# t-taniai/LocalExpStereo

Measured on AMD Instinct MI355X. Metric: Mcost-evals/s (pixels x hypotheses / s), guided-filter cost aggregation, 1500x1000x256 vol, higher is better.
Workload: dtype i32 fixed-point box sums (exact; i64 stage-2 window sums), f32 3x3 algebra and combination

## Files before the change

localexpstereo_amd/csrc/les_hip.hip:

```cpp
#include "../../include/localexp_hip.h"
#include "les_kernels.h"
#include "les_march.h"
#include "les_propose.h"
#include "les_post.h"
#include "les_pairwise.h"
#include "les_fusion.h"
#include "les_eval.h"
#include "les_maxflow.h"
#include "les_maxflow_tiled.h"
#include "les_maxflow_cell.h"
#include "les_bilateral.h"
#include "les_vdisp.h"
#include "les_dense.h"
#include "les_costvol.h"
#include "les_crossview.h"
#include "les_wtavol.h"
#include "les_confidence.h"
#include "les_sgm.h"
#include "les_planefit.h"
#include "les_pyramid.h"
#include "les_speckle.h"
#include "les_reproject.h"

#include "../host/ResidualCut.h"

#include <algorithm>
#include <array>
#include <atomic>
#include <chrono>
#include <cmath>
#include <cstdint>
#include <mutex>
#if !defined(LES_SIM)
#include <dlfcn.h>
#endif
#include <cstdarg>
#include <cstdio>
#include <cstdlib>
#include <cstring>
#include <string>
#include <vector>

namespace {

thread_local std::string g_err;

int fail(int code, const char* fmt, ...)
{
    char buf[512];
    va_list ap;
    va_start(ap, fmt);
    vsnprintf(buf, sizeof buf, fmt, ap);
    va_end(ap);
    g_err = buf;
    return code;
}

enum FallbackReason { FB_RADIUS = 0, FB_NONFINITE, FB_RANGE, FB_THRESHOLD, FB_IMAGE_SIZE, FB_GEOMETRY, FB_PATCHES, FB_GUIDE, FB_COUNT };
void note_fallback(std::atomic<unsigned>& seen, FallbackReason r, const char* fmt, ...)
{
    if (seen.fetch_or(1u << r, std::memory_order_relaxed) & (1u << r)) return;
    static const bool quiet = [] { const char* e = getenv("LES_HIP_QUIET"); return e && atoi(e) != 0; }();
    if (quiet) return;
    char buf[512];
    va_list ap;
    va_start(ap, fmt);
    vsnprintf(buf, sizeof buf, fmt, ap);
    va_end(ap);
    fprintf(stderr, "localexp_hip: strip kernel instead of the march kernel: %s (LES_HIP_QUIET=1 silences this note)\n", buf);
}

#define HIPCHECK(expr)                                                                               \
    do {                                                                                             \
        hipError_t e_ = (expr);                                                                      \
        if (e_ != hipSuccess)                                                                        \
            return fail(LES_HIP_ERR_DEVICE, "%s failed: %s (%s:%d)", #expr, hipGetErrorString(e_), __FILE__, __LINE__); \
    } while (0)

#include "les_hip_march_tables.inc"

struct ViewData {
    float* vol = nullptr;
    bool own_vol = false;
    float4* stats = nullptr;
    uint32_t* ipk = nullptr;
    uint32_t* ipk10 = nullptr;
    float4* feat = nullptr;
    uint32_t* ipk8 = nullptr;
    float* mstats = nullptr;
    float* vol_t = nullptr;
    bool march_ok = false;
    unsigned dmax_bits = 0;
    les::MarchView mv = {};
    les::MarchView mv2 = {};
    float lo2 = 0.0f;
    bool march2_ok = false;
};

}

#include "les_hip_mem.h"

struct MtHost;
namespace { void mt_host_free(MtHost* m); }
struct WtaVol;
namespace { void wtavol_free(WtaVol* w); }
struct SgmWork;
namespace { void sgm_free(SgmWork* w); }
struct FitTables;
namespace { void fit_tables_free(FitTables* t); }

namespace {

struct VdispGroup { int c0, c1, slices; };
struct UnaryTables {
    int n = 0;
    DevBuf<char> mem;
    const les::Job* d_jobs = nullptr; int njobs = 0;
    const les::Job* d_mjobs = nullptr; int nmgroups = 0;
    const MarchEntry* mentry = nullptr;
    bool march_ok = false;
    const les::RawCall* d_rawcalls = nullptr; const long long* d_raw_off = nullptr;
    long long raw_floats = 0; int raw_chunks = 1;
    const les::WtaJob* d_targets = nullptr; const long long* d_out_off = nullptr; int out_stride = 0;
    const les::BfJob* d_bfjobs = nullptr; int nbfjobs = 0, bf_np = 1;
    std::vector<VdispGroup> vd_groups;
    const les::RawCall* d_vd_calls = nullptr;
    const float4* d_vd_stand_in = nullptr;
    int vd_max_slices = 0, vd_chunks = 1;
};

struct UnaryWorkspace {
    bool shared = false;
    struct Slot {
        DevBuf<float> raw;
        DevBuf<unsigned> flags;
        DevBuf<les::Job> rjobs;
        DevBuf<float> vol;
    } slot[2];
};

}

struct les_hip_ctx {
    les_hip_params p;
    int filter = LES_HIP_FILTER_GF;
    int R;
    DevBuf<float> d_bf_tab;
    const StripEntry* strip;
    const StripEntry* istrip[2] = {nullptr, nullptr};
    int interp = 1;
    const MarchEntry* march = nullptr;
    int ncu = 256;
    std::atomic<unsigned> fallback_seen{0};
    hipStream_t stream;
    les::Geom geom;
    ViewData v[2];
    float naive_alpha = 0;
    float naive_th_grad = 0;
    int naive = 0;
    float th_color = 0, th_grad = 0;
    float max_vdisp = 0.0f, random_vdisp = 0.0f;
    float4* d_planes = nullptr; size_t planes_cap = 0;
    DevBuf<float> d_map;
    DevBuf<les::WtaJob> d_wta;
    DevBuf<float4> d_wta_planes;
    DevBuf<float> d_pw_tab; float pw_omega = -1.f, pw_epsilon = -1.f;
    std::mutex mu;
    unsigned long long gen = 0;
    std::vector<les_hip_scratch*> idle_scratch;
    bool maxflow_lds_ready = false;
    bool maxflow_tiled_lds_ready = false;
    std::vector<les_hip_scratch*> own_scratch;
    WtaVol* wtavol = nullptr;
    SgmWork* sgm = nullptr;
    FitTables* fit_tables = nullptr;
    DevBuf<long long> mesh_ws[2];
    std::vector<MtHost*> mt_idle;
    ~les_hip_ctx()
    {
        for (ViewData& w : v) {
            if (w.own_vol && w.vol) (void)hipFree(w.vol);
            for (void* q : {(void*)w.stats, (void*)w.ipk, (void*)w.ipk10, (void*)w.feat, (void*)w.ipk8, (void*)w.mstats, (void*)w.vol_t})
                if (q) (void)hipFree(q);
        }
        if (d_planes) (void)hipFree(d_planes);
    }
};

struct les_hip_batch {
    int n = 0, R = 0;
    UnaryTables tab;
    mutable UnaryWorkspace ws;
    std::vector<les_hip_rect> targets;
    int device = 0;
    DevBuf<les::Rect4> d_units;
    DevBuf<les::WtaJob> d_targets;
    DevBuf<float> rs_disp; DevBuf<int> rs_idx, rs_noi, rs_no; DevBuf<uint64_t> rs_state; DevBuf<float> rs_refit; DevBuf<les::RansacCell> rs_cell;
    les::RansacScratch rs = {nullptr, nullptr, nullptr, nullptr, nullptr, nullptr, 0, nullptr};
    int wta_chunks = 1;
    int graph_chunks = 1;
    std::vector<long long> graph_off;
    long long graph_nodes = 0;
    DevBuf<long long> d_graph_off;
    DevBuf<double> d_flow0;
    mutable std::mutex mt_mu;
    mutable DevBuf<les::MtTile> d_mt_tiles;
    mutable DevBuf<int> d_mt_tiles_per_cell;
    mutable int mt_ntiles = -1;
    mutable std::mutex mf_mu;
    mutable DevBuf<int> d_mf_list;
    mutable int mf_list_key = -1;
    mutable int mf_count[3] = {0, 0, 0};
    mutable std::mutex re_mu;
    mutable DevBuf<double> d_region_part[2];
    mutable int region_chunks = -1;
};

struct les_hip_scratch {
    les_hip_ctx* c = nullptr;
    hipStream_t stream = nullptr;
    DevBuf<float> d_tile; PinnedBuf<float> h_tile;
    DevBuf<float4> d_plane; PinnedBuf<float4> h_plane;
    struct Entry { les_hip_rect f, t; UnaryTables tab; unsigned long long stamp; };
    std::vector<Entry> cache;
    unsigned long long clock = 0;
    UnaryWorkspace ws;
};

namespace {

std::atomic<unsigned long long> g_ctx_gen{0};
std::mutex g_live_mu;
std::vector<std::pair<unsigned long long, les_hip_ctx*>> g_live;
void release_hidden_scratch(unsigned long long gen, les_hip_scratch* s)
{
    std::lock_guard<std::mutex> lk(g_live_mu);
    for (auto& e : g_live)
        if (e.first == gen) {
            std::lock_guard<std::mutex> lk2(e.second->mu);
            e.second->idle_scratch.push_back(s);
            return;
        }
}
thread_local unsigned long long tl_stream_gen = 0;
thread_local hipStream_t tl_stream = nullptr;
inline hipStream_t cur_stream(const les_hip_ctx* c) { return (tl_stream_gen != 0 && tl_stream_gen == c->gen) ? tl_stream : c->stream; }

#include "les_hip_march.inc"

float naive_alpha(const les_hip_ctx* c) { return c->naive_alpha; }

#include "les_hip_vdisp.inc"
#include "les_hip_bilateral.inc"
#include "les_hip_unary.inc"

}

#include "les_hip_context.inc"
#include "les_hip_batch.inc"
#include "les_hip_cuts.inc"
#include "les_hip_eval.inc"
#include "les_hip_speckle.inc"
#include "les_hip_ingest_post.inc"
#include "les_hip_exchange.inc"
#include "les_hip_dense.inc"
#include "les_hip_costvol.inc"
#include "les_hip_crossview.inc"
#include "les_hip_wtavol.inc"
#include "les_hip_confidence.inc"
#include "les_hip_sgm.inc"
#include "les_hip_planefit.inc"
#include "les_hip_pyramid.inc"
#include "les_hip_reproject.inc"
```

localexpstereo_amd/csrc/les_hip_march.inc:

```
int check_rects(const les_hip_ctx* c, const les_hip_rect& f, const les_hip_rect& t)
{
    if (f.w < 0 || f.h < 0 || t.w < 0 || t.h < 0) return fail(LES_HIP_ERR_ARG, "negative rect size");
    if (f.x < 0 || f.y < 0 || f.x + f.w > c->p.W || f.y + f.h > c->p.H) return fail(LES_HIP_ERR_ARG, "filterRect outside the image");
    if (t.w > 0 && t.h > 0 && (t.x < f.x || t.y < f.y || t.x + t.w > f.x + f.w || t.y + t.h > f.y + f.h))
        return fail(LES_HIP_ERR_ARG, "targetRect not inside filterRect");
    return LES_HIP_OK;
}

int build_jobs(const les_hip_ctx* c, int n, const les_hip_rect* frs, const les_hip_rect* trs, int out_slabs,
               std::vector<les::Job>& jobs)
{
    const int TW = c->strip->TW, R = c->R;
    const long long P = (long long)c->p.H * c->p.W;
    long long strips = 0;
    for (int i = 0; i < n; i++) {
        int rc = check_rects(c, frs[i], trs[i]);
        if (rc) return rc;
        if (trs[i].w > 0 && trs[i].h > 0) strips += (trs[i].w + TW - 1) / TW;
    }
    int max_rows = 1 << 30;
    if (strips > 0 && strips < 2048) {
        long long want = (2048 + strips - 1) / strips;
        int tallest = 0;
        for (int i = 0; i < n; i++) tallest = std::max(tallest, trs[i].h);
        max_rows = std::max<long long>(std::max(8 * R, 64), (tallest + want - 1) / want);
    }
    jobs.clear();
    for (int i = 0; i < n; i++) {
        const les_hip_rect &f = frs[i], &t = trs[i];
        if (t.w <= 0 || t.h <= 0) continue;
        for (int sy = 0; sy < t.h; sy += max_rows)
            for (int sx = 0; sx < t.w; sx += TW) {
                les::Job j;
                j.tx0 = t.x + sx; j.ty0 = t.y + sy;
                j.tw = std::min(TW, t.w - sx); j.th = std::min(max_rows, t.h - sy);
                j.cx0 = f.x; j.cy0 = f.y; j.cx1 = f.x + f.w; j.cy1 = f.y + f.h;
                j.out_off = (out_slabs ? (long long)(i / out_slabs) * P : 0) + (long long)j.ty0 * c->p.W + j.tx0;
                j.out_stride = c->p.W;
                j.plane_idx = i;
                jobs.push_back(j);
            }
    }
    std::stable_sort(jobs.begin(), jobs.end(), [](const les::Job& a, const les::Job& b) {
        if (a.tx0 != b.tx0) return a.tx0 < b.tx0;
        if (a.ty0 != b.ty0) return a.ty0 < b.ty0;
        return a.plane_idx < b.plane_idx;
    });
    return LES_HIP_OK;
}

bool build_march_jobs(les_hip_ctx* c, int n, const les_hip_rect* frs, const les_hip_rect* trs, int out_slabs,
                      std::vector<les::Job>& jobs, bool& ok, const MarchEntry*& entry)
{
    jobs.clear();
    ok = false;
    entry = nullptr;
    if (!c->march) return true;
    const int R = c->R, W = c->p.W, H = c->p.H;
    const long long P = (long long)H * W;
    ok = true;
    for (int i = 0; i < n; i++) {
        const les_hip_rect &f = frs[i], &t = trs[i];
        if (t.w <= 0 || t.h <= 0) continue;
        if ((f.x > 0 && t.x - f.x < 2 * R) || (f.x + f.w < W && (f.x + f.w) - (t.x + t.w) < 2 * R) ||
            (f.y > 0 && t.y - f.y < 2 * R) || (f.y + f.h < H && (f.y + f.h) - (t.y + t.h) < 2 * R)) ok = false;
    }
    if (!ok) {
        note_fallback(c->fallback_seen, FB_GEOMETRY, "a target rectangle lies closer than 2 x radius = %d pixels to a filterRect border that is not an image border", 2 * R);
        return true;
    }
    const int ncu = c->ncu;
    const MarchEntry* cands[2] = {c->march, find_march(c->R, 0)};
    const MarchEntry* m = c->march;
    int max_rows = 1 << 30;
    {
        double best = 1e300;
        const int row_opts[] = {1 << 30, 1024, 512, 384, 256, 192, 128, 96, 64, 48, 32};
        for (int g = 0; g < 2; g++) {
            const MarchEntry* e = cands[g];
            if (!e || (g == 1 && e == cands[0])) continue;
            if (const char* w = getenv("LES_HIP_MARCH_WIDE")) if ((atoi(w) != 0) != (g == 0)) continue;
            for (int ro : row_opts) {
                long long njobs = 0;
                int rows = 0, useful = 0;
                for (int i = 0; i < n; i++) {
                    const les_hip_rect& t = trs[i];
                    if (t.w <= 0 || t.h <= 0) continue;
                    const int ns = (t.w + e->TW - 1) / e->TW;
                    const int nr = (t.h + ro - 1) / ro, sh = (t.h + nr - 1) / nr;
                    njobs += (long long)ns * nr;
                    rows = std::max(rows, sh);
                    useful = std::max(useful, (t.w + ns - 1) / ns);
                }
                if (njobs == 0) continue;
                const long long wgs = (njobs + e->NJ - 1) / e->NJ;
                const double ticks = (double)((rows + 4 * R + e->BY - 1) / e->BY + 3);
                const double cost = (double)((wgs + ncu - 1) / ncu) * ticks * (1.0 + 1e-3 * (double)wgs / ncu) + (ro == (1 << 30) ? 0.0 : 1e-6);
                if (cost < best) { best = cost; m = e; max_rows = ro; }
            }
        }
    }
    if (const char* e = getenv("LES_HIP_MARCH_ROWS")) max_rows = std::max(1, atoi(e));
    entry = m;
    const int TW = m->TW, NJ = m->NJ;
    for (int i = 0; i < n; i++) {
        const les_hip_rect &f = frs[i], &t = trs[i];
        if (t.w <= 0 || t.h <= 0) continue;
        const int ns = (t.w + TW - 1) / TW, sw = (t.w + ns - 1) / ns;
        const int nr = (t.h + max_rows - 1) / max_rows, sh = (t.h + nr - 1) / nr;
        for (int sy = 0; sy < t.h; sy += sh)
            for (int sx = 0; sx < t.w; sx += sw) {
                les::Job j;
                j.tx0 = t.x + sx; j.ty0 = t.y + sy;
                j.tw = std::min(sw, t.w - sx); j.th = std::min(sh, t.h - sy);
                j.cx0 = f.x; j.cy0 = f.y; j.cx1 = f.x + f.w; j.cy1 = f.y + f.h;
                j.out_off = (out_slabs ? (long long)(i / out_slabs) * P : 0) + (long long)j.ty0 * W + j.tx0;
                j.out_stride = W;
                j.plane_idx = i;
                jobs.push_back(j);
            }
    }
    std::stable_sort(jobs.begin(), jobs.end(), [](const les::Job& a, const les::Job& b) {
        if (a.tx0 != b.tx0) return a.tx0 < b.tx0;
        if (a.ty0 != b.ty0) return a.ty0 < b.ty0;
        return a.plane_idx < b.plane_idx;
    });
    while (!jobs.empty() && jobs.size() % NJ) {
        les::Job pad = jobs.back();
        pad.tw = 0; pad.th = 0;
        jobs.push_back(pad);
    }
    return true;
}

int ensure_planes(les_hip_ctx* c, size_t n)
{
    if (n <= c->planes_cap) return LES_HIP_OK;
    if (c->d_planes) HIPCHECK(hipFree(c->d_planes));
    c->d_planes = nullptr; c->planes_cap = 0;
    size_t cap = std::max<size_t>(n, 1024);
    HIPCHECK(hipMalloc((void**)&c->d_planes, cap * sizeof(float4)));
    c->planes_cap = cap;
    return LES_HIP_OK;
}

struct RawPatches { const les::RawCall* calls; const long long* off; float* raw; int n, chunks; };

les::View strip_view(const les_hip_ctx* c, int mode)
{
    les::View view{c->v[mode].vol, c->v[mode].stats, c->v[mode].ipk, c->v[mode].ipk10, nullptr, nullptr, mode ? -1.0f : 1.0f, c->th_color, c->th_grad};
    if (c->naive) { view.feat_self = c->v[mode].feat; view.feat_other = c->v[1 - mode].feat; }
    return view;
}

int launch_march(les_hip_ctx* c, const MarchEntry* m, int mode, const les::Job* d_mjobs, int ngroups, const float4* d_planes, float* d_out, int check,
                 hipStream_t stream, const RawPatches* rp = nullptr)
{
    if (ngroups <= 0) return LES_HIP_OK;
    les::MarchView mv = c->v[mode].mv;
    if (c->naive) {
        if (!rp || !rp->raw || !c->v[1 - mode].feat) return fail(LES_HIP_ERR_ARG, "view %d was not supplied at creation", mode);
        hipLaunchKernelGGL(les::les_naive_raw_kernel, dim3(rp->n, rp->chunks), dim3(256), 0, stream, c->geom, strip_view(c, mode), rp->calls, d_planes, rp->raw);
        mv.vol = rp->raw; mv.raw_off = rp->off;
    }
    hipLaunchKernelGGL(m->fn, dim3(ngroups), dim3(m->NT), 0, stream, c->geom, mv, d_mjobs, d_planes, d_out, ngroups, check);
    HIPCHECK(hipGetLastError());
    return LES_HIP_OK;
}

const StripEntry* strip_for(const les_hip_ctx* c) { return (c->naive || c->interp == 1) ? c->strip : c->istrip[c->interp == 0 ? 0 : 1]; }

int launch_strips(les_hip_ctx* c, int mode, const les::Job* d_jobs, int njobs, const float4* d_planes, float* d_out, int check, hipStream_t stream)
{
    if (njobs <= 0) return LES_HIP_OK;
    if (mode < 0 || mode > 1 || !c->v[mode].stats || (c->naive ? !c->v[1 - mode].feat : !c->v[mode].vol))
        return fail(LES_HIP_ERR_ARG, "view %d was not supplied at creation", mode);
    const StripEntry* se = strip_for(c);
    if (!se) return fail(LES_HIP_ERR_UNSUPPORTED, "no strip kernel for interpolation %d at guided-filter radius %d", c->interp, c->R);
    const les::View view = strip_view(c, mode);
    hipLaunchKernelGGL(se->fn, dim3(njobs), dim3(se->NT), 0, stream, c->geom, view, d_jobs, d_planes, d_out, njobs, check);
    HIPCHECK(hipGetLastError());
    return LES_HIP_OK;
}

bool interp_march_ok(const les_hip_ctx* c, int mode)
{
    return !c->naive && c->interp != 1 && c->march && c->v[mode].march_ok && (c->interp == 0 || c->v[mode].march2_ok);
}

int launch_nan_spread(les_hip_ctx* c, int mode, int n, const les::RawCall* calls, const les::WtaJob* targets, const long long* out_off, int stride,
                      const float4* d_planes, const unsigned* flags, float* d_out, int check, hipStream_t stream)
{
    if (n <= 0) return LES_HIP_OK;
    if (c->interp == 2)
        hipLaunchKernelGGL(les::les_nan_spread_kernel<2>, dim3(n), dim3(256), 0, stream, c->geom, (const float*)c->v[mode].vol, calls, targets, out_off, stride,
                           d_planes, flags, d_out, 2 * c->R, check);
    else
        hipLaunchKernelGGL(les::les_nan_spread_kernel<0>, dim3(n), dim3(256), 0, stream, c->geom, (const float*)c->v[mode].vol, calls, targets, out_off, stride,
                           d_planes, flags, d_out, 2 * c->R, check);
    HIPCHECK(hipGetLastError());
    return LES_HIP_OK;
}

int launch_interp_march(les_hip_ctx* c, const MarchEntry* m, int mode, const les::Job* d_mjobs, int ngroups, const RawPatches& rp,
                        unsigned* d_flags, const les::Job* d_sjobs, les::Job* d_rjobs, int nsjobs, const les::WtaJob* targets, const long long* out_off,
                        int stride, const float4* d_planes, float* d_out, int check, hipStream_t stream)
{
    const ViewData& v = c->v[mode];
    const bool quad = c->interp == 2;
    les::MarchView mv = quad ? v.mv2 : v.mv;
    mv.vol = rp.raw; mv.raw_off = rp.off; mv.vol_t = nullptr;
    if (quad) {
        if (!c->istrip[1]) return fail(LES_HIP_ERR_UNSUPPORTED, "no strip kernel for interpolation 2 at guided-filter radius %d", c->R);
        HIPCHECK(hipMemsetAsync(d_flags, 0, (size_t)rp.n * sizeof(unsigned), stream));
        hipLaunchKernelGGL(les::les_interp_raw_kernel<2>, dim3(rp.n, rp.chunks), dim3(256), 0, stream, c->geom, (const float*)v.vol, rp.calls, d_planes,
                           rp.raw, d_flags, v.lo2);
    } else {
        hipLaunchKernelGGL(les::les_interp_raw_kernel<0>, dim3(rp.n, rp.chunks), dim3(256), 0, stream, c->geom, (const float*)v.vol, rp.calls, d_planes,
                           rp.raw, (unsigned*)nullptr, -INFINITY);
    }
    HIPCHECK(hipGetLastError());
    if (ngroups > 0) hipLaunchKernelGGL(m->fn, dim3(ngroups), dim3(m->NT), 0, stream, c->geom, mv, d_mjobs, d_planes, d_out, ngroups, check);
    HIPCHECK(hipGetLastError());
    if (quad && nsjobs > 0) {
        hipLaunchKernelGGL(les::les_mask_jobs_kernel, dim3((nsjobs + 255) / 256), dim3(256), 0, stream, d_sjobs, d_rjobs, (const unsigned*)d_flags, nsjobs);
        HIPCHECK(hipGetLastError());
        const StripEntry* se = c->istrip[1];
        hipLaunchKernelGGL(se->fn, dim3(nsjobs), dim3(se->NT), 0, stream, c->geom, strip_view(c, mode), (const les::Job*)d_rjobs, d_planes, d_out, nsjobs, check);
        HIPCHECK(hipGetLastError());
        return launch_nan_spread(c, mode, rp.n, rp.calls, targets, out_off, stride, d_planes, d_flags, d_out, check, stream);
    }
    return LES_HIP_OK;
}

float naive_alpha(const les_hip_ctx* c);

int build_march_view(les_hip_ctx* c, int m, const double* d_hs)
{
    ViewData& v = c->v[m];
    const size_t P = (size_t)c->p.H * c->p.W;
    const int W = c->p.W, H = c->p.H;
    v.march_ok = false;
    v.march2_ok = false;
    if ((unsigned long long)P * (4ull * les::kMarchStatWords) >= (1ull << 31)) {
        note_fallback(c->fallback_seen, FB_IMAGE_SIZE, "image of %d x %d pixels (32-bit row offsets reach 2^26 pixels)", W, H);
        return LES_HIP_OK;
    }
    const float th = c->naive ? c->th_color + c->th_grad : c->p.th_col;
    if (!(th > 0.0f) || !(th < INFINITY)) { note_fallback(c->fallback_seen, FB_THRESHOLD, "truncation threshold %g is not positive and finite", (double)th); return LES_HIP_OK; }
    if (d_hs) {
        unsigned dbits = 0;
        struct DevBuf { void* p = nullptr; ~DevBuf() { if (p) (void)hipFree(p); } } dm;
        HIPCHECK(hipMalloc(&dm.p, sizeof(unsigned)));
        unsigned* d_dmax = static_cast<unsigned*>(dm.p);
        HIPCHECK(hipMemsetAsync(d_dmax, 0, sizeof(unsigned), cur_stream(c)));
        HIPCHECK(hipMalloc((void**)&v.ipk8, P * sizeof(uint32_t)));
        HIPCHECK(hipMalloc((void**)&v.mstats, P * les::kMarchStatWords * sizeof(float)));
        hipLaunchKernelGGL(les::les_march_stats_kernel, dim3((W + 255) / 256, H), dim3(256), 0, cur_stream(c), d_hs, v.ipk, v.ipk8, v.mstats, d_dmax, H, W, c->R, c->p.eps);
        HIPCHECK(hipGetLastError());
        HIPCHECK(hipMemcpyAsync(&dbits, d_dmax, sizeof(unsigned), hipMemcpyDeviceToHost, cur_stream(c)));
        HIPCHECK(hipStreamSynchronize(cur_stream(c)));
        v.dmax_bits = dbits;
    }
    auto drop_tiled = [&]() { if (v.vol_t) { (void)hipFree(v.vol_t); v.vol_t = nullptr; } };
    const int nb = 2048;
    std::vector<float> hmin(nb, 0.0f); std::vector<int> hbad(nb, 0);
    if (!c->naive) {
        struct DevBuf { void* p = nullptr; ~DevBuf() { if (p) (void)hipFree(p); } } part;
        HIPCHECK(hipMalloc(&part.p, nb * (sizeof(float) + sizeof(int))));
        float* d_min = static_cast<float*>(part.p);
        int* d_bad = reinterpret_cast<int*>(d_min + nb);
        hipLaunchKernelGGL(les::les_range_kernel, dim3(nb), dim3(256), 0, cur_stream(c), v.vol, P * (size_t)c->p.D, d_min, d_bad);
        HIPCHECK(hipGetLastError());
        HIPCHECK(hipMemcpyAsync(hmin.data(), d_min, nb * sizeof(float), hipMemcpyDeviceToHost, cur_stream(c)));
        HIPCHECK(hipMemcpyAsync(hbad.data(), d_bad, nb * sizeof(int), hipMemcpyDeviceToHost, cur_stream(c)));
        HIPCHECK(hipStreamSynchronize(cur_stream(c)));
    }
    float vmin = INFINITY; int bad = 0;
    for (int i = 0; i < nb; i++) { vmin = std::min(vmin, hmin[i]); bad |= hbad[i]; }
    if (bad || !(vmin < INFINITY)) {
        note_fallback(c->fallback_seen, FB_NONFINITE, "the cost volume of view %d holds NaN or infinite entries", m);
        drop_tiled();
        return LES_HIP_OK;
    }
    vmin = std::min(vmin, 0.5f * th);
    const double range = (double)th - (double)vmin;
    if (!(range <= 8.0 * (double)th)) {
        note_fallback(c->fallback_seen, FB_RANGE, "view %d: costs reach %g below the truncation threshold %g (more than 8 x the threshold)", m, range, (double)th);
        drop_tiled();
        return LES_HIP_OK;
    }
    const unsigned dbits = v.dmax_bits;
    float dmax;
    memcpy(&dmax, &dbits, sizeof dmax);
    if (!(dmax > 0.0f) || !(dmax < INFINITY)) { note_fallback(c->fallback_seen, FB_GUIDE, "view %d: the inverse covariance of the guide is not positive and finite (largest diagonal entry %g)", m, (double)dmax); return LES_HIP_OK; }
    const int K = 2 * c->R + 1;
    auto scaled_view = [&](float lo) {
        const double range = (double)th - (double)lo;
        const double Ba = 0.5 * range * std::sqrt((double)dmax), Bb = range + 1.5 * Ba;
        const double scale = 1073741824.0 / ((double)K * Bb * 1.25);
        const int PB = les::march_pb(c->R);
        const float spf = (float)((double)((1 << PB) - 1) / range);
        const double c0 = std::rint(-(double)lo * (double)spf) - (double)(1 << (PB - 1));
        const double up = 1.0 / (double)spf;
        les::MarchView mv;
        mv.vol = v.vol; mv.ipk8 = v.ipk8; mv.mstats = v.mstats;
        mv.sp = spf;
        mv.pmagic = (float)(12582912.0 + c0);
        mv.poff = (float)(-c0 * up);
        mv.kapS = (float)((double)(1 << les::kMarchSH) * up / 255.0 * scale);
        mv.upS = (float)(up * scale);
        mv.qscale = (float)((double)(1 << les::kMarchS2) / (255.0 * scale));
        mv.kmu = (float)(1.0 / ((double)(1ll << les::kMarchMB) * 255.0));
        mv.raw_off = nullptr;
        mv.vol_t = nullptr;
        return mv;
    };
    les::MarchView mv = scaled_view(vmin);
    if (!c->naive) {
        const float lo2 = (float)((double)vmin - 0.5 * range);
        if ((double)th - (double)lo2 <= 8.0 * (double)th) {
            v.mv2 = scaled_view(lo2);
            v.lo2 = lo2;
            v.march2_ok = true;
        }
    }
    if (!c->naive && v.vol) {
        const char* e = getenv("LES_HIP_TILED");
        const unsigned long long nt = (unsigned long long)H * (unsigned long long)((W + 7) / 8) * 8ull * (unsigned long long)c->p.D;
        if (!(e && atoi(e) == 0) && (unsigned long long)((W + 7) / 8) * (unsigned long long)c->p.D * 32ull < (1ull << 31)) {
            if (v.vol_t) { (void)hipFree(v.vol_t); v.vol_t = nullptr; }
            size_t mem_free = 0, mem_total = 0;
            const bool room = hipMemGetInfo(&mem_free, &mem_total) == hipSuccess && mem_free >= 2 * nt * sizeof(float) + (4ull << 30);
            if (room && hipMalloc((void**)&v.vol_t, nt * sizeof(float)) == hipSuccess) {
                hipLaunchKernelGGL(les::les_tile_volume_kernel, dim3((unsigned)(((W + 7) / 8 * 8 + 63) / 64), (unsigned)H), dim3(256), 0, cur_stream(c), v.vol, v.vol_t, c->p.D, H, W);
                HIPCHECK(hipGetLastError());
                mv.vol_t = v.vol_t;
            } else {
                (void)hipGetLastError();
                v.vol_t = nullptr;
            }
        }
    }
    v.mv = mv;
    v.march_ok = true;
    return LES_HIP_OK;
}

int build_view(les_hip_ctx* c, int m, const uint8_t* im, const float* vol)
{
    const size_t P = (size_t)c->p.H * c->p.W;
    ViewData& v = c->v[m];
    if (vol) {
        if (c->p.volumes_on_device) { v.vol = const_cast<float*>(vol); v.own_vol = false; }
        else {
            HIPCHECK(hipMalloc((void**)&v.vol, P * c->p.D * sizeof(float)));
            v.own_vol = true;
            HIPCHECK(hipMemcpy(v.vol, vol, P * c->p.D * sizeof(float), hipMemcpyHostToDevice));
        }
    }
    if (!im) return LES_HIP_OK;
    uint8_t* d_img = nullptr;
    double* d_hs = nullptr;
    HIPCHECK(hipMalloc((void**)&d_img, P * 3));
    HIPCHECK(hipMemcpy(d_img, im, P * 3, hipMemcpyHostToDevice));
    HIPCHECK(hipMalloc((void**)&v.ipk, P * sizeof(uint32_t)));
    HIPCHECK(hipMalloc((void**)&v.ipk10, P * sizeof(uint32_t)));
    HIPCHECK(hipMalloc((void**)&v.stats, (P * 3 + 1) * sizeof(float4)));
    HIPCHECK(hipMemsetAsync(v.stats + P * 3, 0, sizeof(float4), cur_stream(c)));
    HIPCHECK(hipMalloc((void**)&d_hs, P * 9 * sizeof(double)));
    const int W = c->p.W, H = c->p.H;
    if (c->naive) {
        HIPCHECK(hipMalloc((void**)&v.feat, P * sizeof(float4)));
        hipLaunchKernelGGL(les::les_naive_features_kernel, dim3((c->p.W + 255) / 256, c->p.H), dim3(256), 0, cur_stream(c), d_img, v.feat, c->p.H, c->p.W, naive_alpha(c));
    }
    hipLaunchKernelGGL(les::les_pack_guide_kernel, dim3((unsigned)((P + 255) / 256)), dim3(256), 0, cur_stream(c), d_img, v.ipk, v.ipk10, (int)P);
    hipLaunchKernelGGL(les::les_stats_hsum_kernel, dim3((W + 255) / 256, H), dim3(256), 0, cur_stream(c), v.ipk, d_hs, H, W, c->R);
    hipLaunchKernelGGL(les::les_stats_finish_kernel, dim3((W + 255) / 256, H), dim3(256), 0, cur_stream(c), d_hs, v.stats, H, W, c->R, c->p.eps);
    HIPCHECK(hipGetLastError());
    if (c->march && (v.vol || c->naive)) {
        int rc = build_march_view(c, m, d_hs);
        if (rc) { (void)hipFree(d_img); (void)hipFree(d_hs); return rc; }
    }
    HIPCHECK(hipStreamSynchronize(cur_stream(c)));
    HIPCHECK(hipFree(d_img));
    HIPCHECK(hipFree(d_hs));
    return LES_HIP_OK;
}
```

localexpstereo_amd/csrc/les_hip_march_tables.inc:

```
typedef void (*StripKernel)(les::Geom, les::View, const les::Job*, const float4*, float*, int, int);
struct StripEntry { int R; int variant; int TW; int NT; StripKernel fn; };

#define LES_STRIP_ENTRY(R_, V_, WA_, BY_, SEG_, MW_) \
    { R_, V_, les::StripCfg<R_, WA_, BY_, SEG_>::TW, les::StripCfg<R_, WA_, BY_, SEG_>::NT, les::les_strip_kernel<R_, WA_, BY_, SEG_, MW_> }
const StripEntry kStrips[] = {
    LES_STRIP_ENTRY(1, 0, 64, 16, 4, 2), LES_STRIP_ENTRY(2, 0, 64, 16, 4, 2), LES_STRIP_ENTRY(3, 0, 64, 16, 4, 2),
    LES_STRIP_ENTRY(4, 0, 64, 16, 4, 2), LES_STRIP_ENTRY(5, 0, 64, 16, 4, 2), LES_STRIP_ENTRY(6, 0, 64, 16, 4, 2),
    LES_STRIP_ENTRY(7, 0, 64, 16, 4, 2), LES_STRIP_ENTRY(8, 0, 64, 16, 4, 2), LES_STRIP_ENTRY(9, 0, 64, 16, 4, 2),
    LES_STRIP_ENTRY(10, 0, 64, 21, 3, 3), LES_STRIP_ENTRY(12, 0, 64, 16, 4, 2), LES_STRIP_ENTRY(15, 0, 96, 16, 6, 2),
    LES_STRIP_ENTRY(10, 8, 128, 21, 6, 2), LES_STRIP_ENTRY(10, 11, 64, 21, 3, 2),
};
#define LES_NAIVE_ENTRY(R_, WA_, BY_, SEG_, MW_) \
    { R_, 0, les::StripCfg<R_, WA_, BY_, SEG_>::TW, les::StripCfg<R_, WA_, BY_, SEG_>::NT, les::les_strip_kernel<R_, WA_, BY_, SEG_, MW_, 1> }
const StripEntry kNaiveStrips[] = {
    LES_NAIVE_ENTRY(1, 64, 16, 4, 2), LES_NAIVE_ENTRY(2, 64, 16, 4, 2), LES_NAIVE_ENTRY(3, 64, 16, 4, 2), LES_NAIVE_ENTRY(4, 64, 16, 4, 2),
    LES_NAIVE_ENTRY(5, 64, 16, 4, 2), LES_NAIVE_ENTRY(6, 64, 16, 4, 2), LES_NAIVE_ENTRY(7, 64, 16, 4, 2), LES_NAIVE_ENTRY(8, 64, 16, 4, 2),
    LES_NAIVE_ENTRY(9, 64, 16, 4, 2), LES_NAIVE_ENTRY(10, 64, 16, 4, 2), LES_NAIVE_ENTRY(12, 64, 16, 4, 2), LES_NAIVE_ENTRY(15, 96, 16, 6, 2),
};
#define LES_INTERP_ENTRY(R_, WA_, BY_, SEG_, MW_, SRC_) \
    { R_, 0, les::StripCfg<R_, WA_, BY_, SEG_>::TW, les::StripCfg<R_, WA_, BY_, SEG_>::NT, les::les_strip_kernel<R_, WA_, BY_, SEG_, MW_, SRC_> }
#define LES_INTERP_ENTRIES(SRC_) \
    LES_INTERP_ENTRY(1, 64, 16, 4, 2, SRC_), LES_INTERP_ENTRY(2, 64, 16, 4, 2, SRC_), LES_INTERP_ENTRY(3, 64, 16, 4, 2, SRC_), \
    LES_INTERP_ENTRY(4, 64, 16, 4, 2, SRC_), LES_INTERP_ENTRY(5, 64, 16, 4, 2, SRC_), LES_INTERP_ENTRY(6, 64, 16, 4, 2, SRC_), \
    LES_INTERP_ENTRY(7, 64, 16, 4, 2, SRC_), LES_INTERP_ENTRY(8, 64, 16, 4, 2, SRC_), LES_INTERP_ENTRY(9, 64, 16, 4, 2, SRC_), \
    LES_INTERP_ENTRY(10, 64, 16, 4, 2, SRC_), LES_INTERP_ENTRY(12, 64, 16, 4, 2, SRC_), LES_INTERP_ENTRY(15, 96, 16, 6, 2, SRC_)
const StripEntry kNearestStrips[] = { LES_INTERP_ENTRIES(2) };
const StripEntry kQuadraticStrips[] = { LES_INTERP_ENTRIES(3) };
const StripEntry* find_interp_strip(int R, int interp)
{
    for (const auto& e : (interp == 0 ? kNearestStrips : kQuadraticStrips))
        if (e.R == R) return &e;
    return nullptr;
}
const StripEntry* find_naive_strip(int R)
{
    for (const auto& e : kNaiveStrips)
        if (e.R == R) return &e;
    return nullptr;
}
const StripEntry* find_strip(int R)
{
    int variant = 0;
    if (const char* v = getenv("LES_HIP_VARIANT")) variant = atoi(v);
    const StripEntry* def = nullptr;
    for (const auto& e : kStrips) {
        if (e.R != R) continue;
        if (e.variant == variant) return &e;
        if (e.variant == 0) def = &e;
    }
    return def;
}

typedef void (*MarchKernel)(les::Geom, les::MarchView, const les::Job*, const float4*, float*, int, int);
struct MarchEntry { int R; int TW; int NJ; int NT; int BY; MarchKernel fn; };
#define LES_MARCH_ENTRY(R_, WGC_, NJ_, BY_) \
    { R_, les::MarchCfg<R_, WGC_, NJ_, BY_>::TW, NJ_, les::MarchCfg<R_, WGC_, NJ_, BY_>::NT, BY_, les::les_march_kernel<R_, WGC_, NJ_, BY_> }
const MarchEntry kMarch[] = {
    LES_MARCH_ENTRY(10, 256, 1, 7),
#if defined(LES_MARCH_LAB) && defined(LES_MARCH_NARROW_NJ1)
    LES_MARCH_ENTRY(10, 128, 1, 7),
#else
    LES_MARCH_ENTRY(10, 128, 2, 7),
#endif
    LES_MARCH_ENTRY(7, 256, 1, 5),
    LES_MARCH_ENTRY(7, 128, 2, 5),
#if !defined(LES_MARCH_FEW_RADII)
    LES_MARCH_ENTRY(2, 256, 1, 2),  LES_MARCH_ENTRY(2, 128, 2, 2),
    LES_MARCH_ENTRY(3, 256, 1, 3),  LES_MARCH_ENTRY(3, 128, 2, 3),
    LES_MARCH_ENTRY(4, 256, 1, 3),  LES_MARCH_ENTRY(4, 128, 2, 3),
    LES_MARCH_ENTRY(5, 256, 1, 4),  LES_MARCH_ENTRY(5, 128, 2, 4),
    LES_MARCH_ENTRY(6, 256, 1, 5),  LES_MARCH_ENTRY(6, 128, 2, 5),
    LES_MARCH_ENTRY(8, 256, 1, 6),  LES_MARCH_ENTRY(8, 128, 2, 6),
    LES_MARCH_ENTRY(9, 256, 1, 7),  LES_MARCH_ENTRY(9, 128, 2, 7),
#endif
};
const MarchEntry* find_march(int R, int wide = 1)
{
    if (const char* k = getenv("LES_HIP_KERNEL")) if (!strcmp(k, "strip")) return nullptr;
    const MarchEntry* best = nullptr;
    for (const auto& e : kMarch)
        if (e.R == R && (!best || (wide ? e.TW > best->TW : e.TW < best->TW))) best = &e;
    return best;
}

constexpr long long kRawPatchCapFloats = 1ll << 30;
constexpr int kRansacMaxSam = 500;
constexpr int kRansacChunks = 5;
constexpr int kRansacChunkEnds[kRansacChunks] = {16, 64, 128, 256, kRansacMaxSam};
```

localexpstereo_amd/csrc/les_hip_unary.inc:

```

int build_unary_tables(les_hip_ctx* c, int n, const les_hip_rect* frs, const les_hip_rect* trs, int out_slabs, bool compact, UnaryTables& t)
{
    for (int i = 0; i < n; i++) {
        int rc = check_rects(c, frs[i], trs[i]);
        if (rc) return rc;
    }
    t.n = n;
    const long long P = (long long)c->p.H * c->p.W;
    std::vector<les::RawCall> calls((size_t)n);
    std::vector<long long> raw_off((size_t)n), out_off((size_t)n);
    long long amax = 1;
    for (int i = 0; i < n; i++) {
        const les_hip_rect &f = frs[i], &r = trs[i];
        const bool live = r.w > 0 && r.h > 0;
        const long long a = live ? (long long)f.w * f.h : 0;
        calls[i] = les::RawCall{f.x, f.y, live ? f.w : 0, live ? f.h : 0, t.raw_floats};
        raw_off[i] = t.raw_floats;
        out_off[i] = compact ? 0 : (out_slabs ? (long long)(i / out_slabs) * P : 0) + (long long)r.y * c->p.W + r.x;
        t.raw_floats += a; amax = std::max(amax, a);
    }
    t.raw_chunks = (int)std::min<long long>(1024, std::max<long long>(1, (amax + 4095) / 4096));
    t.out_stride = compact ? trs[0].w : c->p.W;
    std::vector<les::Job> jobs, mjobs;
    std::vector<les::BfJob> bfjobs;
    std::vector<les::RawCall> vd_calls;
    std::vector<float4> vd_stand;
    if (c->filter == LES_HIP_FILTER_GF) {
        int rc = build_jobs(c, n, frs, trs, out_slabs, jobs);
        if (rc) return rc;
        bool mok = false;
        build_march_jobs(c, n, frs, trs, out_slabs, mjobs, mok, t.mentry);
        t.march_ok = mok && !mjobs.empty();
        if (t.march_ok && c->naive && t.raw_floats > kRawPatchCapFloats) {
            t.march_ok = false;
            note_fallback(c->fallback_seen, FB_PATCHES, "the raw-cost patches of one batch of the image-based energy exceed 4 GB");
        }
        if (!t.march_ok) mjobs.clear();
        if (compact)
            for (auto* v : {&jobs, &mjobs})
                for (les::Job& j : *v) { j.out_off = (long long)(j.ty0 - trs[0].y) * trs[0].w + (j.tx0 - trs[0].x); j.out_stride = trs[0].w; }
        if (c->naive) vdisp_layout(c, n, frs, trs, t, vd_calls, vd_stand);
    } else {
        if (t.raw_floats > kRawPatchCapFloats)
            return fail(LES_HIP_ERR_UNSUPPORTED, "the raw-cost patches of one batch exceed 4 GB (%lld floats): split the batch", t.raw_floats);
        int rc = build_bf_jobs(c, n, frs, trs, out_slabs, compact, bfjobs, t.bf_np);
        if (rc) return rc;
    }
    t.njobs = (int)jobs.size();
    t.nmgroups = t.march_ok ? (int)(mjobs.size() / t.mentry->NJ) : 0;
    t.nbfjobs = (int)bfjobs.size();
    std::vector<char> blob;
    auto put = [&](const auto& v) -> size_t {
        if (v.empty()) return SIZE_MAX;
        const size_t off = (blob.size() + 255) & ~(size_t)255, bytes = v.size() * sizeof(v[0]);
        blob.resize(off + bytes);
        memcpy(blob.data() + off, v.data(), bytes);
        return off;
    };
    static_assert(sizeof(les::WtaJob) == sizeof(les_hip_rect), "rect layout");
    const std::vector<les_hip_rect> targets(trs, trs + n);
    const size_t o_jobs = put(jobs), o_mjobs = put(mjobs), o_calls = put(calls), o_raw_off = put(raw_off), o_targets = put(targets),
                 o_out_off = put(out_off), o_bfjobs = put(bfjobs), o_vd_calls = put(vd_calls), o_vd_stand = put(vd_stand);
    if (blob.empty()) return LES_HIP_OK;
    int rc = t.mem.alloc(blob.size());
    if (rc) return rc;
    HIPCHECK(hipMemcpy(t.mem.p, blob.data(), blob.size(), hipMemcpyHostToDevice));
    auto at = [&](size_t off) -> const void* { return off == SIZE_MAX ? nullptr : t.mem.p + off; };
    t.d_jobs = static_cast<const les::Job*>(at(o_jobs));
    t.d_mjobs = static_cast<const les::Job*>(at(o_mjobs));
    t.d_rawcalls = static_cast<const les::RawCall*>(at(o_calls));
    t.d_raw_off = static_cast<const long long*>(at(o_raw_off));
    t.d_targets = static_cast<const les::WtaJob*>(at(o_targets));
    t.d_out_off = static_cast<const long long*>(at(o_out_off));
    t.d_bfjobs = static_cast<const les::BfJob*>(at(o_bfjobs));
    t.d_vd_calls = static_cast<const les::RawCall*>(at(o_vd_calls));
    t.d_vd_stand_in = static_cast<const float4*>(at(o_vd_stand));
    return LES_HIP_OK;
}

int unary_kind(const les_hip_ctx* c, const UnaryTables& t, int mode)
{
    if (c->filter != LES_HIP_FILTER_GF) return 2;
    if (!t.march_ok) return 0;
    if (c->naive || c->interp == 1) return c->march && c->v[mode].march_ok ? 1 : 0;
    return interp_march_ok(c, mode) && t.raw_floats <= kRawPatchCapFloats ? 1 : 0;
}

int run_unary(les_hip_ctx* c, const UnaryTables& t, UnaryWorkspace& w, int mode, const float4* d_planes, float* d_out, int check, hipStream_t stream)
{
    int rc = view_ok(c, mode);
    if (rc) return rc;
    const int kind = unary_kind(c, t, mode);
    const bool patches = kind == 2 || (kind == 1 && (c->naive || c->interp != 1));
    const bool vdisp = kind == 0 && c->naive;
    const bool masked = vdisp || (kind == 1 && !c->naive && c->interp == 2);
    UnaryWorkspace::Slot& s = w.slot[w.shared ? mode : 0];
    if (patches || masked) {
        std::unique_lock<std::mutex> lk(c->mu, std::defer_lock);
        if (w.shared) lk.lock();
        const size_t min_raw = w.shared ? 1 : 256 * 256, min_jobs = w.shared ? 1 : 64;
        if (patches) rc = s.raw.grow((size_t)std::max<long long>(t.raw_floats, 1), min_raw, stream);
        if (!rc && masked) rc = s.flags.grow((size_t)std::max(t.n, 1), 1, stream);
        if (!rc && masked) rc = s.rjobs.grow((size_t)std::max(t.njobs, 1), min_jobs, stream);
        if (!rc && vdisp) rc = s.vol.grow(std::max<size_t>((size_t)t.vd_max_slices * c->p.H * c->p.W, 1), 1, stream);
        if (rc) return rc;
    }
    const RawPatches rp{t.d_rawcalls, t.d_raw_off, s.raw.p, t.n, t.raw_chunks};
    if (kind == 2) return launch_bf(c, mode, t.d_bfjobs, t.nbfjobs, t.bf_np, t.d_rawcalls, t.n, t.raw_chunks, s.raw.p, d_planes, d_out, check, stream);
    if (kind == 1) {
        if (c->naive) return launch_naive_march(c, t.mentry, mode, t.d_mjobs, t.nmgroups, d_planes, d_out, check, stream, rp);
        if (c->interp == 1) return launch_march(c, t.mentry, mode, t.d_mjobs, t.nmgroups, d_planes, d_out, check, stream);
        return launch_interp_march(c, t.mentry, mode, t.d_mjobs, t.nmgroups, rp, s.flags.p, t.d_jobs, s.rjobs.p, t.njobs, t.d_targets, t.d_out_off,
                                   t.out_stride, d_planes, d_out, check, stream);
    }
    if (!c->naive && c->interp != 1 && t.march_ok && interp_march_ok(c, mode))
        note_fallback(c->fallback_seen, FB_PATCHES, "the raw-cost patches of one batch at interpolation %d exceed 4 GB", c->interp);
    rc = launch_strips(c, mode, t.d_jobs, t.njobs, d_planes, d_out, check, stream);
    if (rc) return rc;
    if (vdisp) return launch_vdisp_strips(c, t, s.vol.p, s.flags.p, s.rjobs.p, mode, d_planes, d_out, check, stream);
    if (!c->naive && c->interp != 1)
        return launch_nan_spread(c, mode, t.n, t.d_rawcalls, t.d_targets, t.d_out_off, t.out_stride, d_planes, nullptr, d_out, check, stream);
    return LES_HIP_OK;
}
```

localexpstereo_amd/csrc/les_hip_vdisp.inc:

```

void launch_naive_raw(les_hip_ctx* c, int mode, const les::RawCall* calls, int n, int chunks, const float4* d_planes, float* raw, hipStream_t stream)
{
    hipLaunchKernelGGL(les::les_naive_raw_v_kernel, dim3(n, chunks), dim3(256), 0, stream, c->geom, strip_view(c, mode), calls, d_planes, raw, 0, 0,
                       (unsigned*)nullptr);
}

int launch_naive_march(les_hip_ctx* c, const MarchEntry* m, int mode, const les::Job* d_mjobs, int ngroups, const float4* d_planes, float* d_out, int check,
                       hipStream_t stream, const RawPatches& rp)
{
    if (ngroups <= 0) return LES_HIP_OK;
    if (!rp.raw || !c->v[1 - mode].feat) return fail(LES_HIP_ERR_ARG, "view %d was not supplied at creation", mode);
    launch_naive_raw(c, mode, rp.calls, rp.n, rp.chunks, d_planes, rp.raw, stream);
    les::MarchView mv = c->v[mode].mv;
    mv.vol = rp.raw; mv.raw_off = rp.off;
    hipLaunchKernelGGL(m->fn, dim3(ngroups), dim3(m->NT), 0, stream, c->geom, mv, d_mjobs, d_planes, d_out, ngroups, check);
    HIPCHECK(hipGetLastError());
    return LES_HIP_OK;
}

constexpr long long kVdispVolCapFloats = 1ll << 28;

void vdisp_layout(const les_hip_ctx* c, int n, const les_hip_rect* frs, const les_hip_rect* trs, UnaryTables& t, std::vector<les::RawCall>& calls,
                  std::vector<float4>& stand)
{
    const long long HW = (long long)c->p.H * c->p.W;
    const int cap = (int)std::max<long long>(1, kVdispVolCapFloats / std::max<long long>(HW, 1));
    calls.resize((size_t)n);
    stand.resize((size_t)n);
    std::vector<std::vector<les_hip_rect>> used;
    VdispGroup g{0, 0, 0};
    long long amax = 1;
    for (int i = 0; i < n; i++) {
        const les_hip_rect f = frs[i];
        const bool live = trs[i].w > 0 && trs[i].h > 0 && f.w > 0 && f.h > 0;
        int s = 0;
        if (live) {
            auto overlaps = [&](const les_hip_rect& r) { return f.x < r.x + r.w && r.x < f.x + f.w && f.y < r.y + r.h && r.y < f.y + f.h; };
            for (s = 0; s < (int)used.size(); s++) {
                bool free_ = true;
                for (const auto& r : used[s]) if (overlaps(r)) { free_ = false; break; }
                if (free_) break;
            }
            if (s == (int)used.size()) {
                if (s == cap) {
                    g.c1 = i; g.slices = s; t.vd_groups.push_back(g);
                    g = VdispGroup{i, i, 0};
                    used.clear(); s = 0;
                }
                used.emplace_back();
            }
            used[s].push_back(f);
            amax = std::max(amax, (long long)f.w * f.h);
        }
        calls[i] = les::RawCall{f.x, f.y, live ? f.w : 0, live ? f.h : 0, (long long)s * HW + (long long)f.y * c->p.W + f.x};
        stand[i] = make_float4(0.0f, 0.0f, (float)s, 0.0f);
    }
    g.c1 = n; g.slices = (int)used.size(); t.vd_groups.push_back(g);
    for (const auto& gg : t.vd_groups) t.vd_max_slices = std::max(t.vd_max_slices, gg.slices);
    t.vd_chunks = (int)std::min<long long>(1024, std::max<long long>(1, (amax + 4095) / 4096));
}

int launch_vdisp_strips(les_hip_ctx* c, const UnaryTables& t, float* vol, unsigned* flags, les::Job* rjobs, int mode, const float4* d_planes,
                        float* d_out, int check, hipStream_t stream)
{
    const int njobs = t.njobs;
    if (njobs <= 0 || t.n <= 0 || t.vd_max_slices <= 0) return LES_HIP_OK;
    const StripEntry* se = find_interp_strip(c->R, 0);
    if (!se || se->TW < c->strip->TW)
        return fail(LES_HIP_ERR_UNSUPPORTED, "no nearest-slice strip kernel for guided-filter radius %d (vertical disparity on the strip path)", c->R);
    les::Geom g = c->geom;
    g.D0 = 0; g.th_col = INFINITY;
    les::View view = strip_view(c, mode);
    view.vol = vol;
    const les::RawCall* vd_calls = t.d_vd_calls;
    const les::Job* jobs = t.d_jobs;
    const float4* stand_in = t.d_vd_stand_in;
    for (const auto& gr : t.vd_groups) {
        if (gr.c1 <= gr.c0 || gr.slices <= 0) continue;
        g.D = gr.slices;
        if (t.vd_groups.size() > 1) HIPCHECK(hipMemsetAsync(flags, 0, (size_t)t.n * sizeof(unsigned), stream));
        hipLaunchKernelGGL(les::les_naive_raw_v_kernel, dim3(gr.c1 - gr.c0, t.vd_chunks), dim3(256), 0, stream, c->geom, strip_view(c, mode),
                           vd_calls + gr.c0, d_planes + gr.c0, vol, c->p.W, 1, flags + gr.c0);
        hipLaunchKernelGGL(les::les_mask_jobs_kernel, dim3((njobs + 255) / 256), dim3(256), 0, stream, jobs, rjobs, (const unsigned*)flags, njobs);
        hipLaunchKernelGGL(se->fn, dim3(njobs), dim3(se->NT), 0, stream, g, view, (const les::Job*)rjobs, stand_in, d_out, njobs, 0);
        if (check)
            hipLaunchKernelGGL(les::les_vdisp_check_kernel, dim3(njobs), dim3(256), 0, stream, c->geom, (const les::Job*)rjobs, d_planes, d_out, njobs);
        HIPCHECK(hipGetLastError());
    }
    return LES_HIP_OK;
}
```

localexpstereo_amd/csrc/les_march.h:

```cpp
#pragma once

#include "les_kernels.h"

#if defined(LES_MARCH_LAB)
#include "les_march_lab.h"
#else
#define LES_MARCH_ROLE_ORDER 5
#define LES_STATS_POLICY ""
#define LES_LAB_ROLE_ON(bit) true
#define LES_LAB_ABLATE(bit) false
#endif
#ifndef LES_TICK_BEGIN
#define LES_TICK_BEGIN() ((void)0)
#define LES_TICK_MARK() ((void)0)
#define LES_TICK_BARRIER() __syncthreads()
#define LES_TICK_END(role_) ((void)0)
#endif

namespace les {

constexpr int kMarchSH = 5;
constexpr int kMarchMB = 24;
constexpr int kMarchSL = 3;
constexpr int kMarchS2 = 4;
constexpr int kMarchMagicBits = 0x4B400000;
static_assert(kMarchSH + kMarchMB + kMarchSL == 32, "N cov = t - hi32(M * (s << SL)) needs the scales to meet at 2^32");
__host__ __device__ constexpr int march_pb(int R) { return (2 * R + 1) * (2 * R + 1) < 512 ? 20 : 19; }
#ifndef LES_MARCH_STAT_WORDS
#define LES_MARCH_STAT_WORDS 9
#endif
constexpr int kMarchStatWords = LES_MARCH_STAT_WORDS;
static_assert(kMarchStatWords == 9 || kMarchStatWords == 12, "statistics record of 36 or 48 bytes");

struct MarchView {
    const float* vol;
    const uint32_t* ipk8;
    const float* mstats;
    float sp;
    float pmagic;
    float poff;
    float kapS;
    float upS;
    float qscale;
    float kmu;
    const long long* raw_off;
    const float* vol_t;
};
#ifndef LES_TILED_MIN_SLOPE_WIDE
#define LES_TILED_MIN_SLOPE_WIDE 0.05f
#endif
#ifndef LES_TILED_MIN_SLOPE
#define LES_TILED_MIN_SLOPE 0.125f
#endif

template <int R, int WGC, int NJ, int BY>
struct MarchCfg {
    static constexpr int KS = 2 * R + 1;
    static constexpr int RS = 3 * BY;
    static constexpr int TW = WGC - 4 * R;
    static constexpr int HWV = WGC / 64;
    static constexpr int NW = 3 * HWV * NJ;
    static constexpr int NT = 64 * NW;
    static constexpr int SEGL = 8;
    static constexpr int PADW = 16;
    static constexpr int PCOLS0 = 1 + WGC + WGC / PADW;
    static constexpr int PCOLS = PCOLS0 + ((4 - PCOLS0 % 8) + 8) % 8;
    static_assert(RS >= KS, "the ring must hold a whole window (the row that leaves it is the one written KS rows ago)");
    static_assert(RS - KS < BY, "a ring longer than the window by a block or more wastes registers: pick the smallest block height");
    static_assert(WGC % 64 == 0, "a job slot is a whole number of waves");
    static_assert(BY * (64 / SEGL) <= 64, "one wave prefixes its own tile");
    static_assert(TW > 0, "job too narrow for this radius");
    static_assert(2 * R + 1 < 64, "a window crosses at most one wave boundary");
    static_assert((long long)KS * KS * (1ll << (march_pb(R) - 1 + kMarchSL)) < (1ll << 31), "stage-1 window sums (shifted for the product with M) must fit int32");
    static_assert((long long)KS * 128 * (1ll << (march_pb(R) - 1)) < (1ll << 31), "vertical sums of Iq * pi must fit int32");
    static_assert((long long)KS * (1ll << (30 - kMarchS2)) < (1ll << 31), "the stage-2 window sums, rounded to 2^S2, must fit int32");
    __host__ __device__ static constexpr int pcol(int ci) { return 1 + ci + ci / PADW; }
};

__device__ __forceinline__ void march_prefix_scan8(int4 (&v)[8])
{
#pragma unroll
    for (int j = 1; j < 8; j++) { v[j].x += v[j - 1].x; v[j].y += v[j - 1].y; v[j].z += v[j - 1].z; v[j].w += v[j - 1].w; }
    int4 inc = v[7];
#if defined(LES_SIM) || defined(LES_MARCH_SCAN_PLAIN)
#define LES_SCAN_STEP(N) { inc.x += dpp_row_shr<N>(inc.x); inc.y += dpp_row_shr<N>(inc.y); inc.z += dpp_row_shr<N>(inc.z); inc.w += dpp_row_shr<N>(inc.w); }
    LES_SCAN_STEP(2) LES_SCAN_STEP(4) LES_SCAN_STEP(8)
#undef LES_SCAN_STEP
#else
#define LES_SCAN_ROW(N) "v_add_u32_dpp %0, %0, %0 row_shr:" #N " row_mask:0xf bank_mask:0xf bound_ctrl:1\n" \
                        "v_add_u32_dpp %1, %1, %1 row_shr:" #N " row_mask:0xf bank_mask:0xf bound_ctrl:1\n" \
                        "v_add_u32_dpp %2, %2, %2 row_shr:" #N " row_mask:0xf bank_mask:0xf bound_ctrl:1\n" \
                        "v_add_u32_dpp %3, %3, %3 row_shr:" #N " row_mask:0xf bank_mask:0xf bound_ctrl:1\n"
    asm("s_nop 1\n" LES_SCAN_ROW(2) LES_SCAN_ROW(4) LES_SCAN_ROW(8) : "+v"(inc.x), "+v"(inc.y), "+v"(inc.z), "+v"(inc.w));
#undef LES_SCAN_ROW
#endif
    const int4 off = int4{inc.x - v[7].x, inc.y - v[7].y, inc.z - v[7].z, inc.w - v[7].w};
#pragma unroll
    for (int j = 0; j < 8; j++) { v[j].x += off.x; v[j].y += off.y; v[j].z += off.z; v[j].w += off.w; }
}

template <int BY, int PCOLS>
__device__ __forceinline__ void march_prefix_tile(int4 (*T)[PCOLS], int ci0, int lane)
{
    constexpr int SEGL = 8;
    const int row = 2 * (lane >> 4) + (lane & 1), seg = (lane & 15) >> 1;
    const bool act = row < BY;
    const int c0 = ci0 + seg * SEGL;
    int4* p = &T[act ? row : 0][1 + c0 + c0 / 16];
    int4 v[SEGL];
#pragma unroll
    for (int j = 0; j < SEGL; j++) v[j] = p[j];
    march_prefix_scan8(v);
    if (act) {
#pragma unroll
        for (int j = 0; j < SEGL; j++) lds_store4(&p[j], v[j].x, v[j].y, v[j].z, v[j].w);
    }
}

template <int BY, int PCOLS>
__device__ __forceinline__ void march_prefix_pair(int4 (*TA)[PCOLS], int4 (*TB)[PCOLS], int ci0, int lane)
{
    constexpr int SEGL = 8;
    const int row = 2 * (lane >> 4) + (lane & 1), seg = (lane & 15) >> 1;
    const bool act = row < BY;
    const int c0 = ci0 + seg * SEGL;
    const int pc = 1 + c0 + c0 / 16;
    int4* pa = &TA[act ? row : 0][pc];
    int4* pb = &TB[act ? row : 0][pc];
    int4 va[SEGL], vb[SEGL];
#pragma unroll
    for (int j = 0; j < SEGL; j++) vb[j] = pb[j];
    wave_sync();
#pragma unroll
    for (int j = 0; j < SEGL; j++) va[j] = pa[j];
    LES_MARCH_SCHED_FENCE();
    march_prefix_scan8(vb);
    if (act) {
#pragma unroll
        for (int j = 0; j < SEGL; j++) lds_store4(&pb[j], vb[j].x, vb[j].y, vb[j].z, vb[j].w);
    }
    LES_MARCH_SCHED_FENCE();
    march_prefix_scan8(va);
    if (act) {
#pragma unroll
        for (int j = 0; j < SEGL; j++) lds_store4(&pa[j], va[j].x, va[j].y, va[j].z, va[j].w);
    }
}

#if defined(LES_SIM)
typedef float4 mstat4;
#else
typedef float mstat4 __attribute__((ext_vector_type(4)));
#endif
#if LES_MARCH_STAT_WORDS == 9
typedef float mstat_tail;
#else
typedef mstat4 mstat_tail;
#endif
struct MarchStatRow { mstat4 a, b; mstat_tail c; };
#if defined(LES_SIM) || defined(LES_MARCH_STATS_PLAIN)
struct MarchStatDesc { const char* base; uint32_t bytes; };
__device__ inline MarchStatDesc march_stats_desc(const float* base, uint32_t bytes) { return MarchStatDesc{(const char*)base, bytes}; }
__device__ inline void march_stats_load(MarchStatRow& r, const MarchStatDesc& d, uint32_t voff, uint32_t soff)
{
    const unsigned long long o = (unsigned long long)voff + (unsigned long long)soff;
    float w[8 + sizeof(mstat_tail) / 4];
    for (unsigned i = 0; i < sizeof w / 4; i++) w[i] = (o + 4ull * i + 4 <= d.bytes) ? *reinterpret_cast<const float*>(d.base + o + 4ull * i) : 0.0f;
    memcpy(&r.a, w, 16); memcpy(&r.b, w + 4, 16); memcpy(&r.c, w + 8, sizeof r.c);
}
template <int N>
__device__ inline void march_stats_wait(MarchStatRow& r) { (void)r; }
template <int N>
__device__ inline void march_stats_wait(MarchStatRow& r, MarchStatRow& q) { (void)r; (void)q; }
#else
typedef int MarchStatDesc __attribute__((ext_vector_type(4)));
__device__ __forceinline__ MarchStatDesc march_stats_desc(const float* base, uint32_t bytes)
{
    const unsigned long long a = (unsigned long long)base;
    MarchStatDesc d;
    d.x = __builtin_amdgcn_readfirstlane((int)(uint32_t)a);
    d.y = __builtin_amdgcn_readfirstlane((int)((uint32_t)(a >> 32) & 0xffffu));
    d.z = __builtin_amdgcn_readfirstlane((int)bytes);
    d.w = 0x00027000;
    return d;
}
__device__ __forceinline__ void march_stats_load(MarchStatRow& r, const MarchStatDesc& d, uint32_t voff, uint32_t soff)
{
    asm volatile("buffer_load_dwordx4 %0, %1, %2, %3 offen" LES_STATS_POLICY : "+v"(r.a) : "v"(voff), "s"(d), "s"(soff));
    asm volatile("buffer_load_dwordx4 %0, %1, %2, %3 offen offset:16" LES_STATS_POLICY : "+v"(r.b) : "v"(voff), "s"(d), "s"(soff));
#if LES_MARCH_STAT_WORDS == 9
    asm volatile("buffer_load_dword %0, %1, %2, %3 offen offset:32" LES_STATS_POLICY : "+v"(r.c) : "v"(voff), "s"(d), "s"(soff));
#else
    asm volatile("buffer_load_dwordx4 %0, %1, %2, %3 offen offset:32" LES_STATS_POLICY : "+v"(r.c) : "v"(voff), "s"(d), "s"(soff));
#endif
}
template <int N>
__device__ __forceinline__ void march_stats_wait(MarchStatRow& r) { asm volatile("s_waitcnt vmcnt(%3)" : "+v"(r.a), "+v"(r.b), "+v"(r.c) : "n"(N)); }
template <int N>
__device__ __forceinline__ void march_stats_wait(MarchStatRow& r, MarchStatRow& q)
{
    asm volatile("s_waitcnt vmcnt(%6)" : "+v"(r.a), "+v"(r.b), "+v"(r.c), "+v"(q.a), "+v"(q.b), "+v"(q.c) : "n"(N));
}
#endif
__device__ __forceinline__ int march_stat_m2(const MarchStatRow& r)
{
#if LES_MARCH_STAT_WORDS == 9
    return __float_as_int(r.c);
#else
    return __float_as_int(r.c.x);
#endif
}

__device__ __forceinline__ bool march_label_surely_valid(const Geom& g, float4 pl, int x0, int x1, int y0, int y1)
{
    const float ax0 = pl.x * (float)x0, ax1 = pl.x * (float)x1, by0 = pl.y * (float)y0, by1 = pl.y * (float)y1;
    const float spread = 5.0f * (fabsf(pl.x) + fabsf(pl.y));
    const float lo = (fminf(ax0, ax1) + fminf(by0, by1)) + pl.z - spread;
    const float hi = (fmaxf(ax0, ax1) + fmaxf(by0, by1)) + pl.z + spread;
    const float mag = fmaxf(fabsf(ax0), fabsf(ax1)) + fmaxf(fabsf(by0), fabsf(by1)) + fabsf(pl.z) + spread;
    const float margin = 1e-5f * mag + 1e-30f;
    return (0.0f * pl.w == 0.0f) && mag < 1e30f && (lo - margin >= g.mind) && (hi + margin <= g.maxd);
}

__device__ __forceinline__ bool march_plane_short_gather(const Geom& g, float4 pl, const Job& job, int R, int* slice_lo)
{
    *slice_lo = 0;
    const unsigned long long HW = (unsigned long long)g.H * (unsigned long long)g.W;
    const bool moderate = fabsf(pl.x) < 1e30f && fabsf(pl.y) < 1e30f && fabsf(pl.z) < 1e30f;
    if (!(moderate && g.mind == 0.0f && g.D0 == 0 && g.maxd == (float)(g.D - 1) && g.D >= 2 && HW < (1ull << 24))) return false;
    if ((unsigned long long)g.D * HW < (1ull << 30)) return true;
    const int x0 = max(job.tx0 - 2 * R, job.cx0), x1 = min(job.tx0 + job.tw + 2 * R, job.cx1) - 1;
    const int y0 = max(job.ty0 - 2 * R, job.cy0), y1 = min(job.ty0 + job.th + 2 * R, job.cy1) - 1;
    if (x1 < x0 || y1 < y0) return false;
    const float ax0 = pl.x * (float)x0, ax1 = pl.x * (float)x1, by0 = pl.y * (float)y0, by1 = pl.y * (float)y1;
    const float lo = (fminf(ax0, ax1) + fminf(by0, by1)) + pl.z, hi = (fmaxf(ax0, ax1) + fmaxf(by0, by1)) + pl.z;
    const float mag = fmaxf(fabsf(ax0), fabsf(ax1)) + fmaxf(fabsf(by0), fabsf(by1)) + fabsf(pl.z);
    const float margin = 1e-5f * mag + 1e-30f;
    if (!((lo - margin >= 0.0f) && (hi + margin < g.maxd))) return false;
    const int s0 = (int)floorf(lo - margin), s1 = (int)floorf(hi + margin) + 1;
    *slice_lo = s0;
    return s0 >= 0 && s1 < g.D && (unsigned long long)(s1 - s0 + 1) * HW < (1ull << 28);
}

template <int R, int WGC, int NJ, int BY>
__global__ void __launch_bounds__(3 * WGC * NJ)
les_march_kernel(Geom g, MarchView view, const Job* __restrict__ jobs, const float4* __restrict__ planes,
                 float* __restrict__ out, int ngroups, int check)
{
    using Cfg = MarchCfg<R, WGC, NJ, BY>;
    constexpr int KS = Cfg::KS, RS = Cfg::RS, NT = Cfg::NT, HWV = Cfg::HWV, PCOLS = Cfg::PCOLS;
    constexpr int UN = 3;

    __shared__ int4 s_T1[2][NJ][BY][PCOLS];
    __shared__ int4 s_T2[3][NJ][BY][PCOLS];
    __shared__ float s_rtab[KS + 1];

    int grp;
    {
        const int nwg = (int)gridDim.x, orig = (int)blockIdx.x;
        const int q = nwg / 8, r = nwg % 8, xcd = orig % 8;
        grp = (xcd < r ? xcd * (q + 1) : r * (q + 1) + (xcd - r) * q) + orig / 8;
    }
    if (grp >= ngroups) return;
    const int tid = (int)threadIdx.x;
    const int lane = tid & 63;
    const int wave = readfirstlane_i32(tid >> 6);
    constexpr int kRoleOf[6][3] = {{0, 1, 2}, {2, 1, 0}, {1, 2, 0}, {2, 0, 1}, {1, 0, 2}, {0, 2, 1}};
    const int slot = wave / (3 * HWV), role = kRoleOf[LES_MARCH_ROLE_ORDER][(wave % (3 * HWV)) / HWV], half = wave % HWV;
    const int ci0 = half * 64, ci = ci0 + lane;
    const Job job = jobs[grp * NJ + slot];
    int th_max = 0;
#pragma unroll
    for (int s = 0; s < NJ; s++) th_max = max(th_max, jobs[grp * NJ + s].th);
    const int nblk = (th_max + 4 * R + BY - 1) / BY;
    const int nticks = nblk + 3;
    const int Ttot = job.th > 0 ? job.th + 4 * R : 0;
    const float4 plane = planes[job.plane_idx];
    const int cy1m = max(job.cy1 - 1, job.cy0);

    if (tid <= KS) s_rtab[tid] = tid > 0 ? (float)(1.0 / (double)tid) : 0.0f;
    for (int k = tid; k < 3 * NJ * BY; k += NT) {
        if (k < 2 * NJ * BY) (&s_T1[0][0][0][0])[k * PCOLS] = int4{0, 0, 0, 0};
        (&s_T2[0][0][0][0])[k * PCOLS] = int4{0, 0, 0, 0};
    }
    __syncthreads();

    const int gx = job.tx0 - 2 * R + ci;
    const bool col_in = gx >= job.cx0 && gx < job.cx1 && job.th > 0;
    const int sx = min(max(gx, job.cx0), max(job.cx1 - 1, job.cx0));
    const uint32_t sx4 = (uint32_t)sx * 4u;
    const uint32_t rowB = (uint32_t)g.W * 4u;
    const uint32_t imgB = (uint32_t)g.H * rowB;
    const BufRsrc rs_guide = make_buf(view.ipk8, imgB);
    const int nx = window_count(gx, R, job.cx0, job.cx1);
    const int cP = min(ci + R, WGC - 1), cM = ci - R - 1;
    const int pcP = Cfg::pcol(cP);
    const int pcM = cM >= 0 ? Cfg::pcol(cM) : 0;
    const bool cross = cM >= 0 && (cP >> 6) != (cM >> 6);
    const int pcX = cross ? Cfg::pcol((cP >> 6) * 64 - 1) : 0;
    const int pcS = Cfg::pcol(ci);

    if (role == 0 && LES_LAB_ROLE_ON(1)) {
        const uint32_t HWu = (uint32_t)g.H * (uint32_t)g.W;
        const float g_ax = plane.x * (float)sx;
        const bool fronto = plane.x == 0.0f && plane.y == 0.0f;
        GatherPrep gpc = gather_prepare(g, 0.0f, plane.z, 0u, HWu, true);
        if (gpc.f1 == 0.0f) gpc.i1 = gpc.i0;
        int ringN[RS];
        uint32_t ringG[RS];
#pragma unroll
        for (int k = 0; k < RS; k++) { ringN[k] = 0; ringG[k] = 0u; }
        int Sp = 0;
        int Sc[3] = {1 << (kMarchSH - 1), 1 << (kMarchSH - 1), 1 << (kMarchSH - 1)};
        const uint32_t i0s = (uint32_t)readfirstlane_i32((int)gpc.i0), i1s = (uint32_t)readfirstlane_i32((int)gpc.i1);
        const float f1s = __int_as_float(readfirstlane_i32(__float_as_int(gpc.f1)));
        const int modes = readfirstlane_i32(gpc.mode);
        const float f0s = 1.0f - f1s;
        const bool inv_job = fronto && modes == 2 && !view.raw_off;
        int slice_lo = 0;
        const bool tame = !fronto && !view.raw_off && march_plane_short_gather(g, plane, job, R, &slice_lo);
        const uint32_t W8 = ((uint32_t)g.W + 7u) >> 3;
        const uint32_t trowB = W8 * (uint32_t)g.D * 32u;
        const int trow_lo = max(job.ty0 - 2 * R, job.cy0);
        const int trow_hi = min(job.ty0 - 2 * R + (nblk + 2) * BY, job.cy1);
        const unsigned long long tspanB = (unsigned long long)max(trow_hi - trow_lo, 1) * (unsigned long long)trowB;
        const bool tiled = tame && view.vol_t && fabsf(plane.x) >= (NJ == 1 ? LES_TILED_MIN_SLOPE_WIDE : LES_TILED_MIN_SLOPE) && tspanB < 0xfffffff0ull &&
                           (unsigned long long)W8 * (unsigned long long)g.D * 32ull < (1ull << 31);
        const float spj = !col_in ? 0.0f : (inv_job ? 0.0f : view.sp);
        const float pmj = !col_in ? __int_as_float(kMarchMagicBits) : (inv_job ? fmaf(g.th_col, view.sp, view.pmagic) : view.pmagic);
        auto march_a = [&](auto kind_tag) __attribute__((always_inline)) {
        constexpr int KIND = decltype(kind_tag)::value;
        GatherPrep gp[BY];
        float v0[BY], v1[BY];
        float f1r[BY];
        uint32_t gw[BY];
        uint32_t rowbits = 0, rowbits_nx = 0;
        int nx_rowB = 0;
        float nx_dbase = 0.0f;
        int nx_rowraw = 0;
        int nx_rowT = 0;
        const int fw = job.cx1 - job.cx0;
        const float* v0base = view.vol + (size_t)i0s;
        if constexpr (KIND == 3) v0base = view.vol + view.raw_off[job.plane_idx] - job.cx0;
        if constexpr (KIND == 4) v0base = view.vol + (size_t)slice_lo * (size_t)HWu;
        if constexpr (KIND == 5) v0base = view.vol_t + (size_t)trow_lo * (size_t)(trowB >> 2);
        const unsigned long long rest4 = (unsigned long long)(g.D - slice_lo) * (unsigned long long)imgB;
        const unsigned long long trestB = (unsigned long long)(g.H - trow_lo) * (unsigned long long)trowB;
        const uint32_t tiledB = (uint32_t)(trestB < 0xfffffffcull ? trestB : 0xfffffffcull);
        const BufRsrc rs_v0 = make_buf(v0base, KIND == 3 ? 0xfffffffcu : (KIND == 4 ? (uint32_t)(rest4 < 0xfffffffcull ? rest4 : 0xfffffffcull) : (KIND == 5 ? tiledB : imgB)));
        const uint32_t tcol = (((uint32_t)sx >> 3) * (uint32_t)g.D * 8u + ((uint32_t)sx & 7u)) * 4u;
        const int dsub = g.D0 - slice_lo;
        const BufRsrc rs_v1 = make_buf(view.vol + (size_t)i1s, imgB);
        auto prep = [&](int b) __attribute__((always_inline)) {
            const int t = b * BY + lane;
            const int gy = job.ty0 - 2 * R + t;
            const int sy = min(max(gy, job.cy0), cy1m);
            nx_rowB = (int)((uint32_t)sy * rowB);
            rowbits_nx = ballot_low(t < Ttot && gy >= job.cy0 && gy < job.cy1, BY);
            if constexpr (KIND == 3) nx_rowraw = (sy - job.cy0) * fw * 4;
            else nx_dbase = plane.y * (float)sy + plane.z;
            if constexpr (KIND == 5) nx_rowT = (int)((uint32_t)(sy - trow_lo) * trowB);
        };
        auto issue_row = [&](auto itag) __attribute__((always_inline)) {
            constexpr int i = decltype(itag)::value;
            const uint32_t ro = (uint32_t)readlane_i32(nx_rowB, i);
            if (LES_LAB_ABLATE(64)) { v0[i] = (float)lane; v1[i] = 0.0f; gw[i] = (uint32_t)lane; return; }
            if constexpr (KIND == 3) {
                v0[i] = buf_load<float>(rs_v0, sx4, (uint32_t)readlane_i32(nx_rowraw, i));
            } else if constexpr (KIND < 2) {
                v0[i] = buf_load<float>(rs_v0, sx4, ro);
                if constexpr (KIND == 1) v1[i] = buf_load<float>(rs_v1, sx4, ro);
            } else if constexpr (KIND == 4) {
                const float d = g_ax + readlane_f32(nx_dbase, i);
                const float dc = med3_f32(d, 0.0f, g.maxd);
                const float df = floorf(dc);
                f1r[i] = dc - df;
                const uint32_t e = mad_u24((int)df + dsub, (int)HWu, sx);
                v0[i] = buf_load<float>(rs_v0, e << 2, ro);
                v1[i] = buf_load<float>(rs_v0, (e << 2) + (f1r[i] > 0.0f ? imgB : 0u), ro);
            } else if constexpr (KIND == 5) {
                const float d = g_ax + readlane_f32(nx_dbase, i);
                const float dc = med3_f32(d, 0.0f, g.maxd);
                const float df = floorf(dc);
                f1r[i] = dc - df;
                const uint32_t e = (((uint32_t)(int)df + (uint32_t)g.D0) << 5) + tcol;
                const uint32_t rt = (uint32_t)readlane_i32(nx_rowT, i);
                v0[i] = buf_load<float>(rs_v0, e, rt);
                v1[i] = buf_load<float>(rs_v0, e + (f1r[i] > 0.0f ? 32u : 0u), rt);
            } else {
                const float d_base = readlane_f32(nx_dbase, i);
                const bool inside = col_in && ((rowbits_nx >> i) & 1u);
                gp[i] = gather_prepare(g, g_ax, d_base, (ro >> 2) + (uint32_t)sx, HWu, inside);
                if (gp[i].f1 == 0.0f) gp[i].i1 = gp[i].i0;
                v0[i] = view.vol[gp[i].i0];
                v1[i] = view.vol[gp[i].i1];
            }
            gw[i] = buf_load<uint32_t>(rs_guide, sx4, ro);
        };
        prep(0);
        rowbits = rowbits_nx;
        prep(0);
        static_for<BY>([&](auto itag) { issue_row(itag); });
        LES_TICK_BEGIN();
        for (int k0 = 0; k0 < nticks; k0 += UN) {
            static_for<UN>([&](auto utag) {
                constexpr int BASE = decltype(utag)::value * BY;
                const int k = k0 + decltype(utag)::value;
                if (k < nticks) {
                    if (k < nblk) {
                        int4 (*T)[PCOLS] = s_T1[k & 1][slot];
                        prep(k + 1);
                        static_for<BY>([&](auto itag) {
                            constexpr int i = decltype(itag)::value;
                            constexpr int SLOT = BASE + i;
                            constexpr int OLD = (SLOT + RS - KS) % RS;
                            int pi;
                            if constexpr (KIND == 3) {
                                pi = (__float_as_int(fmaf(v0[i], spj, pmj)) - kMarchMagicBits) & sbfe1(rowbits, i);
                            } else if constexpr (KIND < 2) {
                                float C = v0[i];
                                if constexpr (KIND == 1) C = f0s * v0[i] + f1s * v1[i];
                                const float p = min_f32_finite(C, g.th_col);
                                pi = (__float_as_int(fmaf(p, spj, pmj)) - kMarchMagicBits) & sbfe1(rowbits, i);
                            } else if constexpr (KIND == 4 || KIND == 5) {
                                const float f0 = 1.0f - f1r[i];
                                const float C = f0 * v0[i] + f1r[i] * v1[i];
                                const float p = min_f32_finite(C, g.th_col);
                                pi = (__float_as_int(fmaf(p, spj, pmj)) - kMarchMagicBits) & sbfe1(rowbits, i);
                            } else {
                                const float p = gather_finish(g, gp[i], v0[i], v1[i]);
                                pi = __float_as_int(fmaf(p, view.sp, view.pmagic)) - kMarchMagicBits;
                                pi = gp[i].mode == 3 ? 0 : pi;
                            }
                            const uint32_t gi = gw[i];
                            const int no = ringN[OLD];
                            const uint32_t go = ringG[OLD];
                            ringN[SLOT] = -pi;
                            ringG[SLOT] = gi;
                            Sp = Sp + pi + no;
                            Sc[0] = Sc[0] + mul24_sbyte<0>(gi, pi) + mul24_sbyte<0>(go, no);
                            Sc[1] = Sc[1] + mul24_sbyte<1>(gi, pi) + mul24_sbyte<1>(go, no);
                            Sc[2] = Sc[2] + mul24_sbyte<2>(gi, pi) + mul24_sbyte<2>(go, no);
                            lds_store4(&T[i][pcS], Sp, Sc[0] >> kMarchSH, Sc[1] >> kMarchSH, Sc[2] >> kMarchSH);
                            issue_row(itag);
                        });
                        rowbits = rowbits_nx;
                        LES_TICK_MARK();
                    }
                    {
                        int4 (*TB)[PCOLS] = s_T2[(decltype(utag)::value + UN - 2 % UN) % UN][slot];
                        const bool da = k < nblk, db = !(NJ > 1 && KIND == 2) && k >= 2 && k < nblk + 2;
                        constexpr bool kPair = KIND != 2 && KIND != 4 && KIND != 5;
                        if (kPair && da && db) march_prefix_pair<BY, PCOLS>(s_T1[k & 1][slot], TB, ci0, lane);
                        else {
                            if (da) { wave_sync(); march_prefix_tile<BY, PCOLS>(s_T1[k & 1][slot], ci0, lane); }
                            if (db) march_prefix_tile<BY, PCOLS>(TB, ci0, lane);
                        }
                    }
                    LES_TICK_BARRIER();
                }
            });
        }
        LES_TICK_END(0);
        };
        if (view.raw_off) march_a(std::integral_constant<int, 3>{});
        else if (fronto && f1s == 0.0f) march_a(std::integral_constant<int, 0>{});
        else if (fronto) march_a(std::integral_constant<int, 1>{});
        else if (tiled) march_a(std::integral_constant<int, 5>{});
        else if (tame) march_a(std::integral_constant<int, 4>{});
        else march_a(std::integral_constant<int, 2>{});
    } else if (role == 1 && LES_LAB_ROLE_ON(2)) {
        const bool s1_col = col_in && ci >= R && ci < WGC - R;
        int slice_lo_unused = 0;
        const bool general_plane = !view.raw_off && !(plane.x == 0.0f && plane.y == 0.0f) && !march_plane_short_gather(g, plane, job, R, &slice_lo_unused);
        const float kap_x = s1_col ? view.kapS * s_rtab[nx] : 0.0f;
        const float up_x = s1_col ? view.upS * s_rtab[nx] : 0.0f;
        const uint32_t sxS = (uint32_t)sx * (uint32_t)(4 * kMarchStatWords);
        const uint32_t rowS = (uint32_t)g.W * (uint32_t)(4 * kMarchStatWords);
        const MarchStatDesc ds_stats = march_stats_desc(view.mstats, (uint32_t)g.H * rowS);
        MarchStatRow st[BY];
#pragma unroll
        for (int i = 0; i < BY; i++) {
            st[i].a = st[i].b = mstat4{0.0f, 0.0f, 0.0f, 0.0f};
#if LES_MARCH_STAT_WORDS == 9
            st[i].c = 0.0f;
#else
            st[i].c = mstat4{0.0f, 0.0f, 0.0f, 0.0f};
#endif
        }
        float rny[BY];
        int nx_srow = 0;
        float nx_rny = 0.0f;
        auto prep = [&](int b) __attribute__((always_inline)) {
            const int t = b * BY + lane;
            const int gy1 = job.ty0 - 3 * R + t;
            const bool on = gy1 >= job.cy0 && gy1 < job.cy1 && t >= 2 * R && t < Ttot;
            nx_rny = on ? s_rtab[window_count(gy1, R, job.cy0, job.cy1)] : 0.0f;
            nx_srow = (int)((uint32_t)min(max(gy1, job.cy0), cy1m) * rowS);
        };
        auto issue_row = [&](auto itag) __attribute__((always_inline)) {
            constexpr int i = decltype(itag)::value;
            rny[i] = readlane_f32(nx_rny, i);
            uint32_t soff = (uint32_t)readlane_i32(nx_srow, i) & 0xfffffffcu;
            if (LES_LAB_ABLATE(4)) soff &= 0x3u;
            if (LES_LAB_ABLATE(1)) return;
            march_stats_load(st[i], ds_stats, sxS, soff);
        };
        prep(0);
        static_for<BY>([&](auto itag) { issue_row(itag); });
        LES_TICK_BEGIN();
        for (int k = 0; k < nticks; k++) {
            if (k >= 1 && k <= nblk) {
                const int b = k - 1;
                const int4 (*T1)[PCOLS] = s_T1[b & 1][slot];
                int4 (*T2)[PCOLS] = s_T2[b % 3][slot];
                constexpr int GC = 2, NS = (BY + GC - 1) / GC;
                prep(k);
                int4 pp[2][GC], pm[2][GC], px[2][GC];
                auto lds_stage = [&](auto stag) __attribute__((always_inline)) {
                    constexpr int S = decltype(stag)::value;
#pragma unroll
                    for (int j = 0; j < GC; j++)
                        if (S * GC + j < BY) {
                            if (LES_LAB_ABLATE(2)) { pp[S & 1][j] = int4{lane, k, 2, 3}; pm[S & 1][j] = int4{3, 2, k, lane}; px[S & 1][j] = int4{0, 0, 0, 0}; }
                            else { pp[S & 1][j] = T1[S * GC + j][pcP]; pm[S & 1][j] = T1[S * GC + j][pcM]; px[S & 1][j] = T1[S * GC + j][pcX]; }
                        }
                };
                lds_stage(std::integral_constant<int, 0>{});
                static_for<NS>([&](auto gtag) {
                    constexpr int S = decltype(gtag)::value, CB = S & 1;
                    constexpr int LO = S * GC;
                    constexpr int N = (BY - LO) < GC ? (BY - LO) : GC;
                    if constexpr (S + 1 < NS) lds_stage(std::integral_constant<int, S + 1>{});
                    LES_MARCH_SCHED_FENCE();
                    static_assert(GC == 2, "vmcnt bookkeeping below is written for stages of two rows");
                    if constexpr (N == 2) march_stats_wait<3 * (BY - 2)>(st[LO], st[LO + 1]);
                    else march_stats_wait<3 * (BY - 1)>(st[LO]);
                    static_for<N>([&](auto jtag) {
                        constexpr int j = decltype(jtag)::value;
                        constexpr int i = LO + j;
                        const int s = pp[CB][j].x - pm[CB][j].x + px[CB][j].x;
                        const mstat4 q0 = st[i].a, q1 = st[i].b;
                        const int M0 = __float_as_int(q1.z), M1 = __float_as_int(q1.w), M2 = march_stat_m2(st[i]);
                        const long long s8 = (long long)(s << kMarchSL);
                        const float d0 = (float)((pp[CB][j].y - pm[CB][j].y) + px[CB][j].y + (int)(((long long)M0 * s8 + (1ll << 31)) >> 32));
                        const float d1 = (float)((pp[CB][j].z - pm[CB][j].z) + px[CB][j].z + (int)(((long long)M1 * s8 + (1ll << 31)) >> 32));
                        const float d2 = (float)((pp[CB][j].w - pm[CB][j].w) + px[CB][j].w + (int)(((long long)M2 * s8 + (1ll << 31)) >> 32));
                        const float ka = kap_x * rny[i];
                        const float a0 = fmaf(q0.z, d2, fmaf(q0.y, d1, q0.x * d0)) * ka;
                        const float a1 = fmaf(q1.x, d2, fmaf(q0.w, d1, q0.y * d0)) * ka;
                        const float a2 = fmaf(q1.y, d2, fmaf(q1.x, d1, q0.z * d0)) * ka;
                        const float mp = (float)s * (up_x * rny[i]);
#if LES_MARCH_STAT_WORDS == 9
                        const float bb = fmaf(view.kmu, fmaf(a2, (float)M2, fmaf(a1, (float)M1, a0 * (float)M0)), mp);
#else
                        const float bb = fmaf(-a2, st[i].c.w, fmaf(-a1, st[i].c.z, fmaf(-a0, st[i].c.y, mp)));
#endif
                        lds_store4(&T2[i][pcS], cvt_rpi_i32(a0), cvt_rpi_i32(a1), cvt_rpi_i32(a2), cvt_rpi_i32(bb));
                    });
                    LES_MARCH_SCHED_FENCE();
                    static_for<N>([&](auto jtag) { issue_row(std::integral_constant<int, LO + decltype(jtag)::value>{}); });
                });
                LES_TICK_MARK();
            }
            if (NJ > 1 && general_plane && k >= 2 && k < nblk + 2) march_prefix_tile<BY, PCOLS>(s_T2[(k - 2) % 3][slot], ci0, lane);
            LES_TICK_BARRIER();
        }
        LES_TICK_END(1);
    } else if (role == 2 && LES_LAB_ROLE_ON(4)) {
        const bool out_col = ci >= 2 * R && ci < 2 * R + job.tw && job.th > 0;
        const uint32_t oc4 = (uint32_t)max(ci - 2 * R, 0) * 4u;
        const float vl_xa = (float)gx * plane.x, vl_c = 1.0f * plane.z, vl_zv = 0.0f * plane.w, vl_a5 = plane.x * 5, vl_b5 = plane.y * 5;
        const float c_lane = view.qscale * s_rtab[nx];
        int ring2[4][RS];
#pragma unroll
        for (int k = 0; k < RS; k++) ring2[0][k] = ring2[1][k] = ring2[2][k] = ring2[3][k] = 0;
        long long S2[4] = {1ll << (kMarchS2 - 1), 1ll << (kMarchS2 - 1), 1ll << (kMarchS2 - 1), 1ll << (kMarchS2 - 1)};
        uint32_t gq[BY];
        float rny2[BY];
        uint32_t okbits = 0;
        int nx_grow = 0;
        float nx_rny = 0.0f;
        const BufRsrc rs_out = make_buf(out + job.out_off, 0xfffffffcu);
        const uint32_t ostrideB = (uint32_t)job.out_stride * 4u;
        auto prep = [&](int b) __attribute__((always_inline)) {
            const int t = b * BY + lane;
            const int gy2 = job.ty0 - 4 * R + t;
            nx_rny = s_rtab[window_count(gy2, R, job.cy0, job.cy1)];
            nx_grow = (int)((uint32_t)min(max(gy2, job.cy0), cy1m) * rowB);
            okbits = ballot_low(t >= 4 * R && t < Ttot, BY);
        };
        auto issue_row = [&](auto itag) __attribute__((always_inline)) {
            constexpr int i = decltype(itag)::value;
            rny2[i] = readlane_f32(nx_rny, i);
            if (LES_LAB_ABLATE(128)) { gq[i] = (uint32_t)lane; return; }
            gq[i] = buf_load<uint32_t>(rs_guide, sx4, (uint32_t)readlane_i32(nx_grow, i));
        };
        auto march_d = [&](auto check_tag) __attribute__((always_inline)) {
        constexpr bool CHECK = decltype(check_tag)::value != 0;
        LES_TICK_BEGIN();
        for (int k0 = 0; k0 < nticks; k0 += UN) {
            static_for<UN>([&](auto utag) {
                constexpr int U = decltype(utag)::value;
                constexpr int BASE = ((U + UN - 3 % UN) % UN) * BY;
                const int k = k0 + U;
                if (k < nticks) {
                    if (k >= 3) {
                        const int b = k - 3;
                        const int4 (*T2)[PCOLS] = s_T2[(U + UN - 3 % UN) % UN][slot];
                        constexpr int GD = 1, NS = (BY + GD - 1) / GD;
                        int4 pp[2][GD], pm[2][GD], px[2][GD];
                        auto lds_stage = [&](auto stag) __attribute__((always_inline)) {
                            constexpr int S = decltype(stag)::value;
#pragma unroll
                            for (int j = 0; j < GD; j++)
                                if (S * GD + j < BY) {
                                    if (LES_LAB_ABLATE(16)) { pp[S & 1][j] = int4{lane, b, 2, 3}; pm[S & 1][j] = int4{3, 2, b, lane}; px[S & 1][j] = int4{0, 0, 0, 0}; }
                                    else { pp[S & 1][j] = T2[S * GD + j][pcP]; pm[S & 1][j] = T2[S * GD + j][pcM]; px[S & 1][j] = T2[S * GD + j][pcX]; }
                                }
                        };
                        lds_stage(std::integral_constant<int, 0>{});
                        static_for<NS>([&](auto gtag) {
                            constexpr int S = decltype(gtag)::value, CB = S & 1;
                            constexpr int LO = S * GD;
                            constexpr int N = (BY - LO) < GD ? (BY - LO) : GD;
                            if constexpr (S + 1 < NS) lds_stage(std::integral_constant<int, S + 1>{});
                            LES_MARCH_SCHED_FENCE();
                            static_for<N>([&](auto jtag) {
                                constexpr int j = decltype(jtag)::value;
                                constexpr int i = LO + j;
                                constexpr int SLOT = BASE + i, OLD = (SLOT + RS - KS) % RS;
                                const int h0 = pp[CB][j].x - pm[CB][j].x + px[CB][j].x, h1 = pp[CB][j].y - pm[CB][j].y + px[CB][j].y;
                                const int h2 = pp[CB][j].z - pm[CB][j].z + px[CB][j].z, h3 = pp[CB][j].w - pm[CB][j].w + px[CB][j].w;
                                const int o0 = ring2[0][OLD], o1 = ring2[1][OLD], o2 = ring2[2][OLD], o3 = ring2[3][OLD];
                                ring2[0][SLOT] = h0; ring2[1][SLOT] = h1; ring2[2][SLOT] = h2; ring2[3][SLOT] = h3;
                                acc64_add_i32(S2[0], h0 - o0); acc64_add_i32(S2[1], h1 - o1); acc64_add_i32(S2[2], h2 - o2); acc64_add_i32(S2[3], h3 - o3);
                                if (out_col && ((okbits >> i) & 1u)) {
                                    const int t = b * BY + i;
                                    const uint32_t gi = gq[i];
                                    const float f0 = (float)(int)(S2[0] >> kMarchS2), f1 = (float)(int)(S2[1] >> kMarchS2), f2 = (float)(int)(S2[2] >> kMarchS2), f3 = (float)(int)(S2[3] >> kMarchS2);
                                    const float acc = fmaf(f2, cvt_f32_sbyte<2>(gi), fmaf(f1, cvt_f32_sbyte<1>(gi), fmaf(f0, cvt_f32_sbyte<0>(gi), f3 * 255.0f)));
                                    float q = fmaf(acc * c_lane, rny2[i], view.poff);
                                    if constexpr (CHECK) {
                                        const int gy2 = job.ty0 + t - 4 * R;
                                        const float ds = ((vl_xa + (float)gy2 * plane.y) + vl_c) + vl_zv;
                                        const float dp = ds + vl_a5, dm = ds - vl_a5;
                                        const float d1 = dp + vl_b5, d2 = dp - vl_b5, d3 = dm + vl_b5, d4 = dm - vl_b5;
                                        const float mn = fmin3(fmin3(ds, d1, d2), d3, d4), mx = fmax3(fmax3(ds, d1, d2), d3, d4);
                                        if (!(mn >= g.mind && mx <= g.maxd)) q = LES_COST_INVALID;
                                    }
                                    if (!(LES_LAB_ABLATE(128) && q != 12345.0f))
                                    buf_store<float>(rs_out, oc4, (uint32_t)(t - 4 * R) * ostrideB, q);
                                }
                            });
                            LES_MARCH_SCHED_FENCE();
                        });
                    }
                    if (k >= 2 && k <= nblk + 1) {
                        prep(k - 2);
                        static_for<BY>([&](auto itag) { issue_row(itag); });
                    }
                    LES_TICK_BARRIER();
                }
            });
        }
        LES_TICK_END(2);
        };
        const bool surely_valid = march_label_surely_valid(g, plane, job.tx0, job.tx0 + max(job.tw, 1) - 1, job.ty0, job.ty0 + max(job.th, 1) - 1);
        if (check && !surely_valid) march_d(std::integral_constant<int, 1>{});
        else march_d(std::integral_constant<int, 0>{});
    }
}

__global__ void les_march_stats_kernel(const double* __restrict__ hs, const uint32_t* __restrict__ ipk, uint32_t* __restrict__ ipk8,
                                       float* __restrict__ mstats, unsigned* __restrict__ inv_diag_max, int H, int W, int R, double eps)
{
    int x = (int)(blockIdx.x * blockDim.x + threadIdx.x), y = (int)blockIdx.y;
    if (x >= W) return;
    size_t P = (size_t)H * W;
    double s[9] = {0, 0, 0, 0, 0, 0, 0, 0, 0};
    for (int dy = -R; dy <= R; dy++) {
        int yy = y + dy;
        if (yy < 0 || yy >= H) continue;
        for (int k = 0; k < 9; k++) s[k] += hs[k * P + (size_t)yy * W + x];
    }
    double N = (double)(window_count(x, R, 0, W) * window_count(y, R, 0, H));
    double m0 = s[0] / N, m1 = s[1] / N, m2 = s[2] / N;
    double rr = s[3] / N - m0 * m0 + eps, rg = s[4] / N - m0 * m1, rb = s[5] / N - m0 * m2;
    double gg = s[6] / N - m1 * m1 + eps, gb = s[7] / N - m1 * m2, bb = s[8] / N - m2 * m2 + eps;
    double irr = gg * bb - gb * gb, irg = gb * rb - rg * bb, irb = rg * gb - gg * rb;
    double igg = rr * bb - rb * rb, igb = rb * rg - rr * gb, ibb = rr * gg - rg * rg;
    double det = irr * rr + irg * rg + irb * rb;
    irr /= det; irg /= det; irb /= det; igg /= det; igb /= det; ibb /= det;
    size_t px = (size_t)y * W + x;
    const double fs = (double)(1ll << kMarchMB);
    const double c0 = m0 * 255.0 - 128.0, c1 = m1 * 255.0 - 128.0, c2 = m2 * 255.0 - 128.0;
    const int M0 = (int)fmin(fmax(rint(-c0 * fs), -2147483648.0), 2147483647.0);
    const int M1 = (int)fmin(fmax(rint(-c1 * fs), -2147483648.0), 2147483647.0);
    const int M2 = (int)fmin(fmax(rint(-c2 * fs), -2147483648.0), 2147483647.0);
    float* o = mstats + px * kMarchStatWords;
    o[0] = (float)irr; o[1] = (float)irg; o[2] = (float)irb; o[3] = (float)igg;
    o[4] = (float)igb; o[5] = (float)ibb; o[6] = __int_as_float(M0); o[7] = __int_as_float(M1);
    o[8] = __int_as_float(M2);
    if (kMarchStatWords == 12) { o[9] = (float)(c0 / 255.0); o[10] = (float)(c1 / 255.0); o[11] = (float)(c2 / 255.0); }
    const uint32_t v = ipk[px];
    const uint32_t b0 = ((v & 0xffu) - 128u) & 0xffu, b1 = (((v >> 8) & 0xffu) - 128u) & 0xffu, b2 = (((v >> 16) & 0xffu) - 128u) & 0xffu;
    ipk8[px] = b0 | (b1 << 8) | (b2 << 16);
    const float dmax = fmaxf(fmaxf((float)irr, (float)igg), (float)ibb);
    if (dmax > 0.0f) atomicMax(inv_diag_max, __float_as_uint(dmax));
}

__global__ void les_tile_volume_kernel(const float* __restrict__ src, float* __restrict__ dst, int D, int H, int W)
{
    const int x = (int)(blockIdx.x * 64 + (threadIdx.x & 63)), y = (int)blockIdx.y;
    const int W8 = (W + 7) >> 3;
    if (x >= W8 * 8) return;
    const size_t HW = (size_t)H * W;
    float* o = dst + (((size_t)y * W8 + (size_t)(x >> 3)) * D) * 8 + (x & 7);
    for (int d = (int)(threadIdx.x >> 6); d < D; d += (int)(blockDim.x >> 6))
        o[(size_t)d * 8] = x < W ? src[(size_t)d * HW + (size_t)y * W + x] : 0.0f;
}

__global__ void les_range_kernel(const float* __restrict__ v, size_t n, float* __restrict__ part_min, int* __restrict__ part_bad)
{
    __shared__ float s_min[256];
    __shared__ int s_bad[256];
    float m = INFINITY;
    int bad = 0;
    for (size_t i = (size_t)blockIdx.x * blockDim.x + threadIdx.x; i < n; i += (size_t)gridDim.x * blockDim.x) {
        const float x = v[i];
        if (!(fabsf(x) < INFINITY)) bad = 1;
        else m = fminf(m, x);
    }
    s_min[threadIdx.x] = m; s_bad[threadIdx.x] = bad;
    __syncthreads();
    for (int k = 128; k > 0; k >>= 1) {
        if ((int)threadIdx.x < k) {
            s_min[threadIdx.x] = fminf(s_min[threadIdx.x], s_min[threadIdx.x + k]);
            s_bad[threadIdx.x] |= s_bad[threadIdx.x + k];
        }
        __syncthreads();
    }
    if (threadIdx.x == 0) { part_min[blockIdx.x] = s_min[0]; part_bad[blockIdx.x] = s_bad[0]; }
}

}
```

Baseline: 173,100.

## Chain multiple fronto-parallel march jobs per workgroup with seamless pipeline handoff

Adds a CHAIN variant of the march kernel that runs several consecutive jobs with the same geometry in one workgroup. It overlaps the three-role pipeline across job boundaries, so the fill and drain ticks are paid once per run of jobs instead of once per job. A cost model in build_march_jobs picks the chain length when there are more workgroups than CUs and the target rows cover the whole filter window. This adds per-role lambda specialisation, job-switch resets of the ring state, and extra register and code-size pressure.

```diff
diff --git a/localexpstereo_amd/csrc/les_hip.hip b/localexpstereo_amd/csrc/les_hip.hip
--- a/localexpstereo_amd/csrc/les_hip.hip
+++ b/localexpstereo_amd/csrc/les_hip.hip
@@ -118,6 +118,7 @@
     DevBuf<char> mem;
     const les::Job* d_jobs = nullptr; int njobs = 0;
     const les::Job* d_mjobs = nullptr; int nmgroups = 0;
+    int mchain = 1;
     const MarchEntry* mentry = nullptr;
     bool march_ok = false;
     const les::RawCall* d_rawcalls = nullptr; const long long* d_raw_off = nullptr;
diff --git a/localexpstereo_amd/csrc/les_hip_march.inc b/localexpstereo_amd/csrc/les_hip_march.inc
--- a/localexpstereo_amd/csrc/les_hip_march.inc
+++ b/localexpstereo_amd/csrc/les_hip_march.inc
@@ -50,11 +50,12 @@
 }
 
 bool build_march_jobs(les_hip_ctx* c, int n, const les_hip_rect* frs, const les_hip_rect* trs, int out_slabs,
-                      std::vector<les::Job>& jobs, bool& ok, const MarchEntry*& entry)
+                      std::vector<les::Job>& jobs, bool& ok, const MarchEntry*& entry, int& chain)
 {
     jobs.clear();
     ok = false;
     entry = nullptr;
+    chain = 1;
     if (!c->march) return true;
     const int R = c->R, W = c->p.W, H = c->p.H;
     const long long P = (long long)H * W;
@@ -73,6 +74,11 @@
     const MarchEntry* cands[2] = {c->march, find_march(c->R, 0)};
     const MarchEntry* m = c->march;
     int max_rows = 1 << 30;
+    int forced_chain = -1;
+    if (const char* e = getenv("LES_HIP_MARCH_CHAIN")) forced_chain = std::max(1, atoi(e));
+    bool spans = true;
+    for (int i = 0; i < n; i++)
+        if (trs[i].w > 0 && trs[i].h > 0 && (trs[i].y != frs[i].y || trs[i].h != frs[i].h)) spans = false;
     {
         double best = 1e300;
         const int row_opts[] = {1 << 30, 1024, 512, 384, 256, 192, 128, 96, 64, 48, 32};
@@ -80,7 +86,9 @@
             const MarchEntry* e = cands[g];
             if (!e || (g == 1 && e == cands[0])) continue;
             if (const char* w = getenv("LES_HIP_MARCH_WIDE")) if ((atoi(w) != 0) != (g == 0)) continue;
+            if (forced_chain > 1 && !e->fn_chain && cands[0]->fn_chain) continue;
             for (int ro : row_opts) {
+                if (forced_chain > 1 && ro != (1 << 30)) continue;
                 long long njobs = 0;
                 int rows = 0, useful = 0;
                 for (int i = 0; i < n; i++) {
@@ -96,11 +104,21 @@
                 const long long wgs = (njobs + e->NJ - 1) / e->NJ;
                 const double ticks = (double)((rows + 4 * R + e->BY - 1) / e->BY + 3);
                 const double cost = (double)((wgs + ncu - 1) / ncu) * ticks * (1.0 + 1e-3 * (double)wgs / ncu) + (ro == (1 << 30) ? 0.0 : 1e-6);
-                if (cost < best) { best = cost; m = e; max_rows = ro; }
+                if (cost < best) { best = cost; m = e; max_rows = ro; chain = 1; }
+                if (ro == (1 << 30) && e->fn_chain && spans && wgs > ncu) {
+                    const int chX = (rows + 2 * R + e->BY - 1) / e->BY, LB = (chX * e->BY - R + e->BY - 1) / e->BY;
+                    for (int mm = 2; mm <= 64 && mm <= njobs; mm++) {
+                        const long long grps = (njobs + mm - 1) / mm;
+                        const double cticks = (double)((mm - 1) * LB + chX + 3);
+                        const double ccost = (double)((grps + ncu - 1) / ncu) * cticks * (1.0 + 1e-3 * (double)grps / ncu);
+                        if (ccost < best) { best = ccost; m = e; max_rows = ro; chain = mm; }
+                    }
+                }
             }
         }
     }
     if (const char* e = getenv("LES_HIP_MARCH_ROWS")) max_rows = std::max(1, atoi(e));
+    if (forced_chain >= 1) chain = m->fn_chain ? forced_chain : 1;
     entry = m;
     const int TW = m->TW, NJ = m->NJ;
     for (int i = 0; i < n; i++) {
@@ -125,7 +143,8 @@
         if (a.ty0 != b.ty0) return a.ty0 < b.ty0;
         return a.plane_idx < b.plane_idx;
     });
-    while (!jobs.empty() && jobs.size() % NJ) {
+    chain = (int)std::min<long long>(chain, std::max<long long>((long long)jobs.size(), 1));
+    while (!jobs.empty() && jobs.size() % (chain > 1 ? chain : NJ)) {
         les::Job pad = jobs.back();
         pad.tw = 0; pad.th = 0;
         jobs.push_back(pad);
@@ -153,7 +172,14 @@
     return view;
 }
 
-int launch_march(les_hip_ctx* c, const MarchEntry* m, int mode, const les::Job* d_mjobs, int ngroups, const float4* d_planes, float* d_out, int check,
+void launch_march_kernel(const MarchEntry* m, const les::Geom& geom, const les::MarchView& mv, const les::Job* d_mjobs, int ngroups, int chain,
+                         const float4* d_planes, float* d_out, int check, hipStream_t stream)
+{
+    const MarchKernel fn = chain > 1 ? m->fn_chain : m->fn;
+    hipLaunchKernelGGL(fn, dim3(ngroups), dim3(m->NT), 0, stream, geom, mv, d_mjobs, d_planes, d_out, ngroups, check, chain);
+}
+
+int launch_march(les_hip_ctx* c, const MarchEntry* m, int mode, const les::Job* d_mjobs, int ngroups, int chain, const float4* d_planes, float* d_out, int check,
                  hipStream_t stream, const RawPatches* rp = nullptr)
 {
     if (ngroups <= 0) return LES_HIP_OK;
@@ -163,7 +189,7 @@
         hipLaunchKernelGGL(les::les_naive_raw_kernel, dim3(rp->n, rp->chunks), dim3(256), 0, stream, c->geom, strip_view(c, mode), rp->calls, d_planes, rp->raw);
         mv.vol = rp->raw; mv.raw_off = rp->off;
     }
-    hipLaunchKernelGGL(m->fn, dim3(ngroups), dim3(m->NT), 0, stream, c->geom, mv, d_mjobs, d_planes, d_out, ngroups, check);
+    launch_march_kernel(m, c->geom, mv, d_mjobs, ngroups, chain, d_planes, d_out, check, stream);
     HIPCHECK(hipGetLastError());
     return LES_HIP_OK;
 }
@@ -202,7 +228,7 @@
     return LES_HIP_OK;
 }
 
-int launch_interp_march(les_hip_ctx* c, const MarchEntry* m, int mode, const les::Job* d_mjobs, int ngroups, const RawPatches& rp,
+int launch_interp_march(les_hip_ctx* c, const MarchEntry* m, int mode, const les::Job* d_mjobs, int ngroups, int chain, const RawPatches& rp,
                         unsigned* d_flags, const les::Job* d_sjobs, les::Job* d_rjobs, int nsjobs, const les::WtaJob* targets, const long long* out_off,
                         int stride, const float4* d_planes, float* d_out, int check, hipStream_t stream)
 {
@@ -220,7 +246,7 @@
                            rp.raw, (unsigned*)nullptr, -INFINITY);
     }
     HIPCHECK(hipGetLastError());
-    if (ngroups > 0) hipLaunchKernelGGL(m->fn, dim3(ngroups), dim3(m->NT), 0, stream, c->geom, mv, d_mjobs, d_planes, d_out, ngroups, check);
+    if (ngroups > 0) launch_march_kernel(m, c->geom, mv, d_mjobs, ngroups, chain, d_planes, d_out, check, stream);
     HIPCHECK(hipGetLastError());
     if (quad && nsjobs > 0) {
         hipLaunchKernelGGL(les::les_mask_jobs_kernel, dim3((nsjobs + 255) / 256), dim3(256), 0, stream, d_sjobs, d_rjobs, (const unsigned*)d_flags, nsjobs);
diff --git a/localexpstereo_amd/csrc/les_hip_march_tables.inc b/localexpstereo_amd/csrc/les_hip_march_tables.inc
--- a/localexpstereo_amd/csrc/les_hip_march_tables.inc
+++ b/localexpstereo_amd/csrc/les_hip_march_tables.inc
@@ -51,10 +51,17 @@
     return def;
 }
 
-typedef void (*MarchKernel)(les::Geom, les::MarchView, const les::Job*, const float4*, float*, int, int);
-struct MarchEntry { int R; int TW; int NJ; int NT; int BY; MarchKernel fn; };
+typedef void (*MarchKernel)(les::Geom, les::MarchView, const les::Job*, const float4*, float*, int, int, int);
+struct MarchEntry { int R; int TW; int NJ; int NT; int BY; MarchKernel fn; MarchKernel fn_chain; };
+template <int R_, int WGC_, int NJ_, int BY_>
+constexpr MarchKernel march_chain_fn()
+{
+    if constexpr (NJ_ == 1) return les::les_march_kernel<R_, WGC_, NJ_, BY_, true>;
+    else return nullptr;
+}
 #define LES_MARCH_ENTRY(R_, WGC_, NJ_, BY_) \
-    { R_, les::MarchCfg<R_, WGC_, NJ_, BY_>::TW, NJ_, les::MarchCfg<R_, WGC_, NJ_, BY_>::NT, BY_, les::les_march_kernel<R_, WGC_, NJ_, BY_> }
+    { R_, les::MarchCfg<R_, WGC_, NJ_, BY_>::TW, NJ_, les::MarchCfg<R_, WGC_, NJ_, BY_>::NT, BY_, les::les_march_kernel<R_, WGC_, NJ_, BY_>, \
+      march_chain_fn<R_, WGC_, NJ_, BY_>() }
 const MarchEntry kMarch[] = {
     LES_MARCH_ENTRY(10, 256, 1, 7),
 #if defined(LES_MARCH_LAB) && defined(LES_MARCH_NARROW_NJ1)
diff --git a/localexpstereo_amd/csrc/les_hip_unary.inc b/localexpstereo_amd/csrc/les_hip_unary.inc
--- a/localexpstereo_amd/csrc/les_hip_unary.inc
+++ b/localexpstereo_amd/csrc/les_hip_unary.inc
@@ -29,7 +29,7 @@
         int rc = build_jobs(c, n, frs, trs, out_slabs, jobs);
         if (rc) return rc;
         bool mok = false;
-        build_march_jobs(c, n, frs, trs, out_slabs, mjobs, mok, t.mentry);
+        build_march_jobs(c, n, frs, trs, out_slabs, mjobs, mok, t.mentry, t.mchain);
         t.march_ok = mok && !mjobs.empty();
         if (t.march_ok && c->naive && t.raw_floats > kRawPatchCapFloats) {
             t.march_ok = false;
@@ -47,7 +47,7 @@
         if (rc) return rc;
     }
     t.njobs = (int)jobs.size();
-    t.nmgroups = t.march_ok ? (int)(mjobs.size() / t.mentry->NJ) : 0;
+    t.nmgroups = t.march_ok ? (int)(mjobs.size() / (t.mchain > 1 ? t.mchain : t.mentry->NJ)) : 0;
     t.nbfjobs = (int)bfjobs.size();
     std::vector<char> blob;
     auto put = [&](const auto& v) -> size_t {
@@ -108,9 +108,9 @@
     const RawPatches rp{t.d_rawcalls, t.d_raw_off, s.raw.p, t.n, t.raw_chunks};
     if (kind == 2) return launch_bf(c, mode, t.d_bfjobs, t.nbfjobs, t.bf_np, t.d_rawcalls, t.n, t.raw_chunks, s.raw.p, d_planes, d_out, check, stream);
     if (kind == 1) {
-        if (c->naive) return launch_naive_march(c, t.mentry, mode, t.d_mjobs, t.nmgroups, d_planes, d_out, check, stream, rp);
-        if (c->interp == 1) return launch_march(c, t.mentry, mode, t.d_mjobs, t.nmgroups, d_planes, d_out, check, stream);
-        return launch_interp_march(c, t.mentry, mode, t.d_mjobs, t.nmgroups, rp, s.flags.p, t.d_jobs, s.rjobs.p, t.njobs, t.d_targets, t.d_out_off,
+        if (c->naive) return launch_naive_march(c, t.mentry, mode, t.d_mjobs, t.nmgroups, t.mchain, d_planes, d_out, check, stream, rp);
+        if (c->interp == 1) return launch_march(c, t.mentry, mode, t.d_mjobs, t.nmgroups, t.mchain, d_planes, d_out, check, stream);
+        return launch_interp_march(c, t.mentry, mode, t.d_mjobs, t.nmgroups, t.mchain, rp, s.flags.p, t.d_jobs, s.rjobs.p, t.njobs, t.d_targets, t.d_out_off,
                                    t.out_stride, d_planes, d_out, check, stream);
     }
     if (!c->naive && c->interp != 1 && t.march_ok && interp_march_ok(c, mode))
diff --git a/localexpstereo_amd/csrc/les_hip_vdisp.inc b/localexpstereo_amd/csrc/les_hip_vdisp.inc
--- a/localexpstereo_amd/csrc/les_hip_vdisp.inc
+++ b/localexpstereo_amd/csrc/les_hip_vdisp.inc
@@ -5,7 +5,7 @@
                        (unsigned*)nullptr);
 }
 
-int launch_naive_march(les_hip_ctx* c, const MarchEntry* m, int mode, const les::Job* d_mjobs, int ngroups, const float4* d_planes, float* d_out, int check,
+int launch_naive_march(les_hip_ctx* c, const MarchEntry* m, int mode, const les::Job* d_mjobs, int ngroups, int chain, const float4* d_planes, float* d_out, int check,
                        hipStream_t stream, const RawPatches& rp)
 {
     if (ngroups <= 0) return LES_HIP_OK;
@@ -13,7 +13,7 @@
     launch_naive_raw(c, mode, rp.calls, rp.n, rp.chunks, d_planes, rp.raw, stream);
     les::MarchView mv = c->v[mode].mv;
     mv.vol = rp.raw; mv.raw_off = rp.off;
-    hipLaunchKernelGGL(m->fn, dim3(ngroups), dim3(m->NT), 0, stream, c->geom, mv, d_mjobs, d_planes, d_out, ngroups, check);
+    launch_march_kernel(m, c->geom, mv, d_mjobs, ngroups, chain, d_planes, d_out, check, stream);
     HIPCHECK(hipGetLastError());
     return LES_HIP_OK;
 }
diff --git a/localexpstereo_amd/csrc/les_march.h b/localexpstereo_amd/csrc/les_march.h
--- a/localexpstereo_amd/csrc/les_march.h
+++ b/localexpstereo_amd/csrc/les_march.h
@@ -242,14 +242,37 @@
     return s0 >= 0 && s1 < g.D && (unsigned long long)(s1 - s0 + 1) * HW < (1ull << 28);
 }
 
-template <int R, int WGC, int NJ, int BY>
+#if defined(LES_SIM)
+__device__ inline int march_opaque_lane(int v) { return v; }
+__device__ inline float march_opaque_f32(float v) { return v; }
+#else
+__device__ __forceinline__ float march_opaque_f32(float v) { asm volatile("" : "+v"(v)); return v; }
+__device__ __forceinline__ int march_opaque_lane(int v) { asm volatile("" : "+v"(v)); return v; }
+#endif
+__device__ __forceinline__ bool march_chain_same_geom(const Job& a, const Job& b)
+{
+    return a.tx0 == b.tx0 && a.tw == b.tw && a.ty0 == b.ty0 && a.th == b.th && a.cx0 == b.cx0 && a.cx1 == b.cx1 && a.cy0 == b.cy0 && a.cy1 == b.cy1 &&
+           a.out_stride == b.out_stride;
+}
+__device__ __forceinline__ int march_chain_class(const Geom& g, const MarchView& view, const Job& job, float4 pl, int check)
+{
+    if (view.raw_off || job.th <= 0 || job.ty0 != job.cy0 || job.ty0 + job.th != job.cy1) return -1;
+    if (!(pl.x == 0.0f && pl.y == 0.0f)) return -1;
+    const GatherPrep gp = gather_prepare(g, 0.0f, pl.z, 0u, (uint32_t)g.H * (uint32_t)g.W, true);
+    const bool surely_valid = march_label_surely_valid(g, pl, job.tx0, job.tx0 + max(job.tw, 1) - 1, job.ty0, job.ty0 + max(job.th, 1) - 1);
+    return (gp.f1 == 0.0f ? 0 : 1) + ((check && !surely_valid) ? 2 : 0);
+}
+
+template <int R, int WGC, int NJ, int BY, bool CHAIN = false>
 __global__ void __launch_bounds__(3 * WGC * NJ)
 les_march_kernel(Geom g, MarchView view, const Job* __restrict__ jobs, const float4* __restrict__ planes,
-                 float* __restrict__ out, int ngroups, int check)
+                 float* __restrict__ out, int ngroups, int check, int chain)
 {
     using Cfg = MarchCfg<R, WGC, NJ, BY>;
     constexpr int KS = Cfg::KS, RS = Cfg::RS, NT = Cfg::NT, HWV = Cfg::HWV, PCOLS = Cfg::PCOLS;
     constexpr int UN = 3;
+    static_assert(!CHAIN || NJ == 1, "jobs are chained in the one-job geometry only (the two-job launches are one round)");
+    static_assert(!CHAIN || BY <= R, "role D's epoch offset X - L >= R - BY + 1 must be positive");
 
     __shared__ int4 s_T1[2][NJ][BY][PCOLS];
     __shared__ int4 s_T2[3][NJ][BY][PCOLS];
@@ -263,20 +286,11 @@
     }
     if (grp >= ngroups) return;
     const int tid = (int)threadIdx.x;
-    const int lane = tid & 63;
+    const int lane0 = tid & 63;
     const int wave = readfirstlane_i32(tid >> 6);
     constexpr int kRoleOf[6][3] = {{0, 1, 2}, {2, 1, 0}, {1, 2, 0}, {2, 0, 1}, {1, 0, 2}, {0, 2, 1}};
     const int slot = wave / (3 * HWV), role = kRoleOf[LES_MARCH_ROLE_ORDER][(wave % (3 * HWV)) / HWV], half = wave % HWV;
-    const int ci0 = half * 64, ci = ci0 + lane;
-    const Job job = jobs[grp * NJ + slot];
-    int th_max = 0;
-#pragma unroll
-    for (int s = 0; s < NJ; s++) th_max = max(th_max, jobs[grp * NJ + s].th);
-    const int nblk = (th_max + 4 * R + BY - 1) / BY;
-    const int nticks = nblk + 3;
-    const int Ttot = job.th > 0 ? job.th + 4 * R : 0;
-    const float4 plane = planes[job.plane_idx];
-    const int cy1m = max(job.cy1 - 1, job.cy0);
+    const int ci0 = half * 64;
 
     if (tid <= KS) s_rtab[tid] = tid > 0 ? (float)(1.0 / (double)tid) : 0.0f;
     for (int k = tid; k < 3 * NJ * BY; k += NT) {
@@ -284,6 +298,40 @@
         (&s_T2[0][0][0][0])[k * PCOLS] = int4{0, 0, 0, 0};
     }
     __syncthreads();
+
+    auto run_pass = [&](auto role_tag) __attribute__((always_inline)) {
+    constexpr int ROLE = decltype(role_tag)::value;
+    int jr = 0;
+    do {
+    const int lane = CHAIN ? march_opaque_lane(lane0) : lane0;
+    const int ci = ci0 + lane;
+    const int jbase = CHAIN ? grp * chain + jr : grp * NJ;
+    const Job job = jobs[jbase + slot];
+    if (CHAIN && job.th <= 0) break;
+    const float4 plane = planes[job.plane_idx];
+    int nrun = 1;
+    bool seam = false;
+    if constexpr (CHAIN) {
+        const int cls = march_chain_class(g, view, job, plane, check);
+        seam = cls >= 0;
+        if (seam)
+            while (jr + nrun < chain) {
+                const Job nj = jobs[jbase + nrun];
+                if (!march_chain_same_geom(job, nj) || march_chain_class(g, view, nj, planes[nj.plane_idx], check) != cls) break;
+                nrun++;
+            }
+    }
+    int th_max = 0;
+#pragma unroll
+    for (int s = 0; s < NJ; s++) th_max = max(th_max, jobs[jbase + s].th);
+    const int chX = (job.th + 2 * R + BY - 1) / BY;
+    const int LB = seam ? (chX * BY - R + BY - 1) / BY : (1 << 29);
+    const int XB = seam ? chX - LB : 0;
+    const int toff = seam ? 2 * R : 0;
+    const int nblk = seam ? (nrun - 1) * LB + chX : (th_max + 4 * R + BY - 1) / BY;
+    const int nticks = nblk + 3;
+    const int Ttot = job.th > 0 ? job.th + 4 * R : 0;
+    const int cy1m = max(job.cy1 - 1, job.cy0);
 
     const int gx = job.tx0 - 2 * R + ci;
     const bool col_in = gx >= job.cx0 && gx < job.cx1 && job.th > 0;
@@ -300,7 +348,7 @@
     const int pcX = cross ? Cfg::pcol((cP >> 6) * 64 - 1) : 0;
     const int pcS = Cfg::pcol(ci);
 
-    if (role == 0 && LES_LAB_ROLE_ON(1)) {
+    if ((ROLE < 0 ? role == 0 : ROLE == 0) && LES_LAB_ROLE_ON(1)) {
         const uint32_t HWu = (uint32_t)g.H * (uint32_t)g.W;
         const float g_ax = plane.x * (float)sx;
         const bool fronto = plane.x == 0.0f && plane.y == 0.0f;
@@ -312,10 +360,10 @@
         for (int k = 0; k < RS; k++) { ringN[k] = 0; ringG[k] = 0u; }
         int Sp = 0;
         int Sc[3] = {1 << (kMarchSH - 1), 1 << (kMarchSH - 1), 1 << (kMarchSH - 1)};
-        const uint32_t i0s = (uint32_t)readfirstlane_i32((int)gpc.i0), i1s = (uint32_t)readfirstlane_i32((int)gpc.i1);
-        const float f1s = __int_as_float(readfirstlane_i32(__float_as_int(gpc.f1)));
+        uint32_t i0s = (uint32_t)readfirstlane_i32((int)gpc.i0), i1s = (uint32_t)readfirstlane_i32((int)gpc.i1);
+        float f1s = __int_as_float(readfirstlane_i32(__float_as_int(gpc.f1)));
         const int modes = readfirstlane_i32(gpc.mode);
-        const float f0s = 1.0f - f1s;
+        float f0s = 1.0f - f1s;
         const bool inv_job = fronto && modes == 2 && !view.raw_off;
         int slice_lo = 0;
         const bool tame = !fronto && !view.raw_off && march_plane_short_gather(g, plane, job, R, &slice_lo);
@@ -326,8 +374,8 @@
         const unsigned long long tspanB = (unsigned long long)max(trow_hi - trow_lo, 1) * (unsigned long long)trowB;
         const bool tiled = tame && view.vol_t && fabsf(plane.x) >= (NJ == 1 ? LES_TILED_MIN_SLOPE_WIDE : LES_TILED_MIN_SLOPE) && tspanB < 0xfffffff0ull &&
                            (unsigned long long)W8 * (unsigned long long)g.D * 32ull < (1ull << 31);
-        const float spj = !col_in ? 0.0f : (inv_job ? 0.0f : view.sp);
-        const float pmj = !col_in ? __int_as_float(kMarchMagicBits) : (inv_job ? fmaf(g.th_col, view.sp, view.pmagic) : view.pmagic);
+        float spj = !col_in ? 0.0f : (inv_job ? 0.0f : view.sp);
+        float pmj = !col_in ? __int_as_float(kMarchMagicBits) : (inv_job ? fmaf(g.th_col, view.sp, view.pmagic) : view.pmagic);
         auto march_a = [&](auto kind_tag) __attribute__((always_inline)) {
         constexpr int KIND = decltype(kind_tag)::value;
         GatherPrep gp[BY];
@@ -347,12 +395,39 @@
         const unsigned long long rest4 = (unsigned long long)(g.D - slice_lo) * (unsigned long long)imgB;
         const unsigned long long trestB = (unsigned long long)(g.H - trow_lo) * (unsigned long long)trowB;
         const uint32_t tiledB = (uint32_t)(trestB < 0xfffffffcull ? trestB : 0xfffffffcull);
-        const BufRsrc rs_v0 = make_buf(v0base, KIND == 3 ? 0xfffffffcu : (KIND == 4 ? (uint32_t)(rest4 < 0xfffffffcull ? rest4 : 0xfffffffcull) : (KIND == 5 ? tiledB : imgB)));
+        BufRsrc rs_v0 = make_buf(v0base, KIND == 3 ? 0xfffffffcu : (KIND == 4 ? (uint32_t)(rest4 < 0xfffffffcull ? rest4 : 0xfffffffcull) : (KIND == 5 ? tiledB : imgB)));
         const uint32_t tcol = (((uint32_t)sx >> 3) * (uint32_t)g.D * 8u + ((uint32_t)sx & 7u)) * 4u;
         const int dsub = g.D0 - slice_lo;
-        const BufRsrc rs_v1 = make_buf(view.vol + (size_t)i1s, imgB);
-        auto prep = [&](int b) __attribute__((always_inline)) {
-            const int t = b * BY + lane;
+        BufRsrc rs_v1 = make_buf(view.vol + (size_t)i1s, imgB);
+        auto chain_taps = [&](int pj) __attribute__((always_inline)) {
+            GatherPrep gq = gather_prepare(g, 0.0f, planes[jobs[jbase + pj].plane_idx].z, 0u, HWu, true);
+            if (gq.f1 == 0.0f) gq.i1 = gq.i0;
+            return gq;
+        };
+        auto chain_issue_switch = [&](int pj) __attribute__((always_inline)) {
+            const GatherPrep gq = chain_taps(pj);
+            rs_v0 = make_buf(view.vol + (size_t)(uint32_t)readfirstlane_i32((int)gq.i0), imgB);
+            rs_v1 = make_buf(view.vol + (size_t)(uint32_t)readfirstlane_i32((int)gq.i1), imgB);
+        };
+        auto chain_consume_switch = [&](int pj) __attribute__((always_inline)) {
+            const GatherPrep gq = chain_taps(pj);
+            f1s = __int_as_float(readfirstlane_i32(__float_as_int(gq.f1)));
+            f0s = 1.0f - f1s;
+            const bool inv = readfirstlane_i32(gq.mode) == 2;
+            const float sp_v = march_opaque_f32(inv ? 0.0f : view.sp);
+            const float pm_v = march_opaque_f32(inv ? fmaf(g.th_col, view.sp, view.pmagic) : view.pmagic);
+            const float mg_v = march_opaque_f32(__int_as_float(kMarchMagicBits));
+            spj = !col_in ? 0.0f : sp_v;
+            pmj = !col_in ? mg_v : pm_v;
+            Sp = 0;
+            Sc[0] = Sc[1] = Sc[2] = 1 << (kMarchSH - 1);
+#pragma unroll
+            for (int q = 0; q < RS; q++) ringN[q] = 0;
+        };
+        int lbc = 0, lbp = 1;
+        int pjc = 0, pjp = 0;
+        auto prep = [&](int lb) __attribute__((always_inline)) {
+            const int t = lb * BY + lane + toff;
             const int gy = job.ty0 - 2 * R + t;
             const int sy = min(max(gy, job.cy0), cy1m);
             nx_rowB = (int)((uint32_t)sy * rowB);
@@ -409,7 +484,12 @@
                 if (k < nticks) {
                     if (k < nblk) {
                         int4 (*T)[PCOLS] = s_T1[k & 1][slot];
-                        prep(k + 1);
+                        if constexpr (CHAIN && KIND < 2) {
+                            if (lbc == LB && pjc + 1 < nrun) { lbc = 0; pjc++; chain_consume_switch(pjc); }
+                            if (lbp == LB && pjp + 1 < nrun) { lbp = 0; pjp++; chain_issue_switch(pjp); }
+                            prep(lbp);
+                            lbc++; lbp++;
+                        } else prep(k + 1);
                         static_for<BY>([&](auto itag) {
                             constexpr int i = decltype(itag)::value;
                             constexpr int SLOT = BASE + i;
@@ -469,7 +549,7 @@
         else if (tiled) march_a(std::integral_constant<int, 5>{});
         else if (tame) march_a(std::integral_constant<int, 4>{});
         else march_a(std::integral_constant<int, 2>{});
-    } else if (role == 1 && LES_LAB_ROLE_ON(2)) {
+    } else if ((ROLE < 0 ? role == 1 : ROLE == 1) && LES_LAB_ROLE_ON(2)) {
         const bool s1_col = col_in && ci >= R && ci < WGC - R;
         int slice_lo_unused = 0;
         const bool general_plane = !view.raw_off && !(plane.x == 0.0f && plane.y == 0.0f) && !march_plane_short_gather(g, plane, job, R, &slice_lo_unused);
@@ -491,8 +571,9 @@
         float rny[BY];
         int nx_srow = 0;
         float nx_rny = 0.0f;
-        auto prep = [&](int b) __attribute__((always_inline)) {
-            const int t = b * BY + lane;
+        int lbp = 1, pjp = 0;
+        auto prep = [&](int lb) __attribute__((always_inline)) {
+            const int t = lb * BY + lane + toff;
             const int gy1 = job.ty0 - 3 * R + t;
             const bool on = gy1 >= job.cy0 && gy1 < job.cy1 && t >= 2 * R && t < Ttot;
             nx_rny = on ? s_rtab[window_count(gy1, R, job.cy0, job.cy1)] : 0.0f;
@@ -515,7 +596,11 @@
                 const int4 (*T1)[PCOLS] = s_T1[b & 1][slot];
                 int4 (*T2)[PCOLS] = s_T2[b % 3][slot];
                 constexpr int GC = 2, NS = (BY + GC - 1) / GC;
-                prep(k);
+                if constexpr (CHAIN) {
+                    if (lbp == LB && pjp + 1 < nrun) { lbp = 0; pjp++; }
+                    prep(lbp);
+                    lbp++;
+                } else prep(k);
                 int4 pp[2][GC], pm[2][GC], px[2][GC];
                 auto lds_stage = [&](auto stag) __attribute__((always_inline)) {
                     constexpr int S = decltype(stag)::value;
@@ -567,10 +652,10 @@
             LES_TICK_BARRIER();
         }
         LES_TICK_END(1);
-    } else if (role == 2 && LES_LAB_ROLE_ON(4)) {
+    } else if ((ROLE < 0 ? role == 2 : ROLE == 2) && LES_LAB_ROLE_ON(4)) {
         const bool out_col = ci >= 2 * R && ci < 2 * R + job.tw && job.th > 0;
         const uint32_t oc4 = (uint32_t)max(ci - 2 * R, 0) * 4u;
-        const float vl_xa = (float)gx * plane.x, vl_c = 1.0f * plane.z, vl_zv = 0.0f * plane.w, vl_a5 = plane.x * 5, vl_b5 = plane.y * 5;
+        float vl_xa = (float)gx * plane.x, vl_c = 1.0f * plane.z, vl_zv = 0.0f * plane.w, vl_a5 = plane.x * 5, vl_b5 = plane.y * 5, vl_yb = plane.y;
         const float c_lane = view.qscale * s_rtab[nx];
         int ring2[4][RS];
 #pragma unroll
@@ -581,10 +666,21 @@
         uint32_t okbits = 0;
         int nx_grow = 0;
         float nx_rny = 0.0f;
-        const BufRsrc rs_out = make_buf(out + job.out_off, 0xfffffffcu);
+        BufRsrc rs_out = make_buf(out + job.out_off, 0xfffffffcu);
         const uint32_t ostrideB = (uint32_t)job.out_stride * 4u;
-        auto prep = [&](int b) __attribute__((always_inline)) {
-            const int t = b * BY + lane;
+        int lbc = 0, lbp = 0;
+        int pjc = 0, pjp = 0;
+        auto chain_switch = [&](int pj) __attribute__((always_inline)) {
+            const Job nj = jobs[jbase + pj];
+            const float4 pl = planes[nj.plane_idx];
+            rs_out = make_buf(out + nj.out_off, 0xfffffffcu);
+            vl_xa = (float)gx * pl.x; vl_c = 1.0f * pl.z; vl_zv = 0.0f * pl.w; vl_a5 = pl.x * 5; vl_b5 = pl.y * 5; vl_yb = pl.y;
+#pragma unroll
+            for (int q = 0; q < RS; q++) ring2[0][q] = ring2[1][q] = ring2[2][q] = ring2[3][q] = 0;
+            S2[0] = S2[1] = S2[2] = S2[3] = 1ll << (kMarchS2 - 1);
+        };
+        auto prep = [&](int lb) __attribute__((always_inline)) {
+            const int t = lb * BY + lane + toff;
             const int gy2 = job.ty0 - 4 * R + t;
             nx_rny = s_rtab[window_count(gy2, R, job.cy0, job.cy1)];
             nx_grow = (int)((uint32_t)min(max(gy2, job.cy0), cy1m) * rowB);
@@ -607,6 +703,11 @@
                 if (k < nticks) {
                     if (k >= 3) {
                         const int b = k - 3;
+                        if constexpr (CHAIN) {
+                            if (lbc == LB + XB && pjc + 1 < nrun) { lbc = XB; pjc++; chain_switch(pjc); }
+                        }
+                        const int tb = (CHAIN ? lbc : b) * BY + toff;
+                        if constexpr (CHAIN) lbc++;
                         const int4 (*T2)[PCOLS] = s_T2[(U + UN - 3 % UN) % UN][slot];
                         constexpr int GD = 1, NS = (BY + GD - 1) / GD;
                         int4 pp[2][GD], pm[2][GD], px[2][GD];
@@ -636,14 +737,14 @@
                                 ring2[0][SLOT] = h0; ring2[1][SLOT] = h1; ring2[2][SLOT] = h2; ring2[3][SLOT] = h3;
                                 acc64_add_i32(S2[0], h0 - o0); acc64_add_i32(S2[1], h1 - o1); acc64_add_i32(S2[2], h2 - o2); acc64_add_i32(S2[3], h3 - o3);
                                 if (out_col && ((okbits >> i) & 1u)) {
-                                    const int t = b * BY + i;
+                                    const int t = tb + i;
                                     const uint32_t gi = gq[i];
                                     const float f0 = (float)(int)(S2[0] >> kMarchS2), f1 = (float)(int)(S2[1] >> kMarchS2), f2 = (float)(int)(S2[2] >> kMarchS2), f3 = (float)(int)(S2[3] >> kMarchS2);
                                     const float acc = fmaf(f2, cvt_f32_sbyte<2>(gi), fmaf(f1, cvt_f32_sbyte<1>(gi), fmaf(f0, cvt_f32_sbyte<0>(gi), f3 * 255.0f)));
                                     float q = fmaf(acc * c_lane, rny2[i], view.poff);
                                     if constexpr (CHECK) {
                                         const int gy2 = job.ty0 + t - 4 * R;
-                                        const float ds = ((vl_xa + (float)gy2 * plane.y) + vl_c) + vl_zv;
+                                        const float ds = ((vl_xa + (float)gy2 * vl_yb) + vl_c) + vl_zv;
                                         const float dp = ds + vl_a5, dm = ds - vl_a5;
                                         const float d1 = dp + vl_b5, d2 = dp - vl_b5, d3 = dm + vl_b5, d4 = dm - vl_b5;
                                         const float mn = fmin3(fmin3(ds, d1, d2), d3, d4), mx = fmax3(fmax3(ds, d1, d2), d3, d4);
@@ -657,7 +758,11 @@
                         });
                     }
                     if (k >= 2 && k <= nblk + 1) {
-                        prep(k - 2);
+                        if constexpr (CHAIN) {
+                            if (lbp == LB + XB && pjp + 1 < nrun) { lbp = XB; pjp++; }
+                            prep(lbp);
+                            lbp++;
+                        } else prep(k - 2);
                         static_for<BY>([&](auto itag) { issue_row(itag); });
                     }
                     LES_TICK_BARRIER();
@@ -670,6 +775,13 @@
         if (check && !surely_valid) march_d(std::integral_constant<int, 1>{});
         else march_d(std::integral_constant<int, 0>{});
     }
+    jr += nrun;
+    } while (CHAIN && jr < chain);
+    };
+    if constexpr (!CHAIN) run_pass(std::integral_constant<int, -1>{});
+    else if (role == 0) run_pass(std::integral_constant<int, 0>{});
+    else if (role == 1) run_pass(std::integral_constant<int, 1>{});
+    else run_pass(std::integral_constant<int, 2>{});
 }
 
 __global__ void les_march_stats_kernel(const double* __restrict__ hs, const uint32_t* __restrict__ ipk, uint32_t* __restrict__ ipk8,
```

Result: slower. 171,300 (-1.1%).
